# tum-vision/mem

Hardware: AMD Instinct MI355X
Metric: pretrain samples/sec (ViT-B, 224^2 event voxels) (higher is better)
Workload: dtype bf16; 1 GPU; MEM pretrain ViT-Base/16, 224^2 2-bin event voxels, bf16, batch 256 per GPU (BASELINE configs[1]); step = rasterize 256x30k events + event_norm + masks + ViT fwd/CE/bwd + clip + AdamW; global_batch=256, parallelism=dp1, stochastic_depth=work skipping, optimizer=AdamW as one launch in front of the next forward, last_block_mlp_rows=rows that reach the head

## Files before the change

include/memhip.h:

```cpp
#ifndef MEMHIP_H
#define MEMHIP_H

#include <stddef.h>
#include <stdint.h>

#ifdef __cplusplus
extern "C" {
#endif

#define MEMHIP_ABI_VERSION 10

#define MEMHIP_OK 0
#define MEMHIP_EINVAL (-1)
#define MEMHIP_EWORKSPACE (-2)
#define MEMHIP_ELAUNCH (-3)
#define MEMHIP_EUNSUPPORTED (-4)

typedef void* memhip_stream_t;

int memhip_abi_version(void);
const char* memhip_last_error(void);
const char* memhip_arch(void);
const char* memhip_build_flags(void);
int memhip_set_option(const char* name, int value);
int memhip_get_option(const char* name, int* value);
int memhip_stream_reserve_cus(memhip_stream_t stream, int cus);


typedef struct memhip_event_aug {
  double scale_x, scale_y;
  int32_t time_flip;
  int32_t flip_x;
  int64_t flip_w;
  int32_t shift_x, shift_y;
  int32_t do_filter;
  int32_t filt_w, filt_h;
  int32_t infer;
} memhip_event_aug_t;
#define MEMHIP_AUG_INFER_FLIP_W 1
#define MEMHIP_AUG_INFER_FILT_W 2
#define MEMHIP_AUG_INFER_FILT_H 4

enum { MEMHIP_RASTER_AUTO = 0, MEMHIP_RASTER_SINGLE = 1, MEMHIP_RASTER_BINNED = 2,
       MEMHIP_RASTER_LDS = 3, MEMHIP_RASTER_GLOBAL = 4, MEMHIP_RASTER_GLOBAL_VAR = 5 };
typedef struct memhip_raster_args {
  const double* ev;
  const int64_t* offsets;
  const memhip_event_aug_t* aug;
  const int32_t* dims;
  int32_t B, H, W, time_surface;
  int32_t form;
  int32_t reserved0;
  int64_t n_events;
  uint8_t* out;
  int32_t* status;
  void* workspace;
  size_t workspace_bytes;
} memhip_raster_args_t;
int memhip_rasterize(const memhip_raster_args_t* args, memhip_stream_t stream);

enum { MEMHIP_RASTER_K_COUNT,
       MEMHIP_RASTER_K_FINALIZE,
       MEMHIP_RASTER_K_LDS,
       MEMHIP_RASTER_K_BIN_KEYS,
       MEMHIP_RASTER_K_BIN_ACCUM };
typedef struct memhip_raster_launch {
  int32_t kernel;
  int32_t grid_x, grid_y;
  int32_t block;
  int32_t lds;
} memhip_raster_launch_t;
typedef struct memhip_raster_plan {
  int32_t family;
  int32_t rows_per_band, bands;
  int32_t band_px, nb;
  int32_t bx;
  uint64_t ws_bytes;
  uint64_t off_bins, off_tstat;
  uint64_t off_keys, off_hdr, off_bad_slots;
  uint64_t clear_ws_bytes, clear_status_bytes, clear_out_bytes;
  int32_t count;
  memhip_raster_launch_t l[2];
} memhip_raster_plan_t;
int memhip_rasterize_plan(const memhip_raster_args_t* args, int device_cus, memhip_raster_plan_t* out);

int memhip_aug_resolve(const double* extent, memhip_event_aug_t* aug, int B, int stage, int fixed_h, int fixed_w,
                       int hmax, int wmax, int32_t* dims, int32_t* status, memhip_stream_t stream);

int memhip_events_extent(const double* ev, const int64_t* offsets, const memhip_event_aug_t* aug,
                         int B, double* extent, memhip_stream_t stream);

#define MEMHIP_DT_U8 0
#define MEMHIP_DT_I8 1
#define MEMHIP_DT_U16 2
#define MEMHIP_DT_I16 3
#define MEMHIP_DT_U32 4
#define MEMHIP_DT_I32 5
#define MEMHIP_DT_U64 6
#define MEMHIP_DT_I64 7
#define MEMHIP_DT_F32 8
#define MEMHIP_DT_F64 9
#define MEMHIP_DT_BOOL 10
int memhip_decode_ncaltech101(const uint8_t* raw, int64_t n_bytes, double* ev, memhip_stream_t stream);
int memhip_events_from_columns(const void* x, int x_dtype, const void* y, int y_dtype, const void* t, int t_dtype,
                               const void* p, int p_dtype, int64_t n, double* ev, memhip_stream_t stream);
size_t memhip_events_dsec_workspace(int64_t n);
int memhip_events_dsec(const void* in, int dtype, int64_t n, double y_limit, double* out, int64_t* n_out,
                       void* workspace, size_t workspace_bytes, memhip_stream_t stream);

int memhip_resample_to_f32(const uint8_t* in, const int32_t* dims, int64_t slot_bytes, int fixed_h, int fixed_w, int mode,
                           const int32_t* offs, int B, int OH, int OW, float* out, memhip_stream_t stream);
int memhip_to_uint8(const float* x, int64_t n, uint8_t* y, memhip_stream_t stream);
int memhip_rand_augment_u8(const uint8_t* in, uint8_t* out, const void* ops, int B, int H, int W, memhip_stream_t stream);
int memhip_color_jitter(const void* in, int in_is_u8, int B, int H, int W, const void* params, float* out, int out_chans,
                        memhip_stream_t stream);

#define MEMHIP_EV_RM_TS 1
#define MEMHIP_EV_HOTPIX 2
#define MEMHIP_EV_LOG 4
#define MEMHIP_EV_GAMMA 8
#define MEMHIP_EV_NORMALIZE 16
int memhip_event_norm(const void* in, int in_is_u8, int B, int H, int W, int flags,
                      float num_stds, float gamma, float* out, int out_chans,
                      memhip_stream_t stream);
int memhip_event_norm_topk(const void* in, int in_is_u8, int B, int H, int W, int flags,
                           int num_hot_pixels, float gamma, float* out, int out_chans,
                           uint64_t* hot_keys, memhip_stream_t stream);

int memhip_mt_seed(uint32_t* mt_state, const uint32_t* key, int key_len);
double memhip_mt_random(uint32_t* mt_state);
int memhip_mask_blockwise(uint32_t* mt_state, int H, int W, int num_masking_patches,
                          int min_num_patches, int max_num_patches, double log_aspect_lo,
                          double log_aspect_hi, int n_masks, uint8_t* out);
int memhip_mask_random_location(uint32_t* mt_state, int H, int W, int num_masking_patches,
                                int n_masks, uint8_t* out);

#define MEMHIP_EPI_BIAS_BF16 0
#define MEMHIP_EPI_BIAS_GELU 1
#define MEMHIP_EPI_RESIDUAL 2
#define MEMHIP_EPI_DGELU 3
#define MEMHIP_EPI_F32 4
#define MEMHIP_EPI_PATCH_EMBED 5
#define MEMHIP_EPI_BIAS_GELU_DG 6
#define MEMHIP_EPI_MUL_AUX 7
#define MEMHIP_EPI_RESIDUAL_DROP 8

typedef struct memhip_dropout {
  uint32_t key0, key1;
  uint32_t site;
  uint32_t thr;
  float scale;
  int32_t row0;
} memhip_dropout_t;
int memhip_dropout_mask(const memhip_dropout_t* d, int row0, int rows, int cols, uint8_t* out, memhip_stream_t stream);
int memhip_dropout_rows_f32(const memhip_dropout_t* d, float* x, int64_t ldx, int rows, int D, memhip_stream_t stream);

typedef struct memhip_gemm_args {
  const void* A; const void* B;
  int64_t lda, ldb;
  int32_t M, N, K, epilogue;
  void* out0; int64_t ldo0;
  void* out1; int64_t ldo1;
  const float* bias;
  const float* vec1;
  float* resid; int64_t ldr;
  const void* aux; int64_t ldaux;
  const float* rowmask;
  float keep_prob;
  float colscale; int32_t colscale_n;
  int32_t rows_per_sample;
  int32_t accumulate;
  float* colsum;
  const int32_t* sample_map;
  int32_t colsum_copies;
  int32_t reserved0;
  const memhip_dropout_t* dropout;
} memhip_gemm_args_t;
int memhip_gemm_bf16_nt(const memhip_gemm_args_t* args, memhip_stream_t stream);

#define MEMHIP_NT_128 0
#define MEMHIP_NT_G256 1
#define MEMHIP_NT_P8_256 2
#define MEMHIP_NT_P8_128 3
#define MEMHIP_NT_P8_PAIR 4
typedef struct memhip_nt_launch {
  int32_t kind;
  int32_t row0, rows;
  int32_t tail_rows;
  int32_t guard;
  int32_t copy;
  int32_t grid, tail_grid;
} memhip_nt_launch_t;
typedef struct memhip_nt_plan { int32_t count; memhip_nt_launch_t l[2]; } memhip_nt_plan_t;
int memhip_gemm_bf16_nt_plan(const memhip_gemm_args_t* args, int stream_cus, int device_cus, memhip_nt_plan_t* out);

size_t memhip_gemm_bf16_tn_workspace(int R, int N, int K);
int memhip_gemm_bf16_tn(const void* A, int64_t lda, const void* B, int64_t ldb, int R, int N, int K,
                        float* out, int64_t ldo, int accumulate, void* workspace, size_t workspace_bytes,
                        memhip_stream_t stream);
typedef struct memhip_tn_problem {
  const void* A; int64_t lda;
  const void* B; int64_t ldb;
  float* out; int64_t ldo;
  int32_t R, N, K;
  int32_t reserved0;
} memhip_tn_problem_t;
size_t memhip_gemm_bf16_tn_group_workspace(const memhip_tn_problem_t* problems, int count);
int memhip_gemm_bf16_tn_group(const memhip_tn_problem_t* problems, int count, int accumulate, void* workspace,
                              size_t workspace_bytes, memhip_stream_t stream);

#define MEMHIP_TN_128 0
#define MEMHIP_TN_P8_ATOMIC 1
#define MEMHIP_TN_P8_WS 2
#define MEMHIP_TN_P8_GROUP 3
typedef struct memhip_tn_part {
  int32_t problem;
  int32_t tiles, splits, rows_per_split;
  int32_t wg_begin, quad_begin;
  int64_t ws_offset;
} memhip_tn_part_t;
typedef struct memhip_tn_launch {
  int32_t kind;
  int32_t count;
  int32_t grid, reduce_grid;
  int32_t memset_first;
  int32_t use_atomics;
  int64_t ws_bytes;
  memhip_tn_part_t p[4];
} memhip_tn_launch_t;
typedef struct memhip_tn_plan { int32_t count; int32_t reserved0; memhip_tn_launch_t l[4]; } memhip_tn_plan_t;
int memhip_gemm_bf16_tn_plan(const memhip_tn_problem_t* problems, int count, int accumulate, const void* workspace,
                             size_t workspace_bytes, int stream_cus, memhip_tn_plan_t* out_plan);
size_t memhip_gemm_bf16_tn_plan_workspace(const memhip_tn_problem_t* problems, int count, int device_cus);
int memhip_colsum_bf16(const void* in, int64_t ld, int R, int C, float* out, memhip_stream_t stream);
int memhip_colsum_fold(float* ws, int copies, int N, float* out, memhip_stream_t stream);

int memhip_residual_rows(const float* x, int64_t ldx, const int32_t* rows, const void* y, int64_t ldy, const float* gamma,
                         const float* rowkeep, float keep_prob, int R, int D, float* out, int64_t ldo,
                         memhip_stream_t stream);
int memhip_scatter_rows_f32(const float* src, int64_t lds, const int32_t* rows, int R, int D, float* dst, int64_t ldd,
                            memhip_stream_t stream);

int memhip_layernorm_fwd(const float* x, int64_t ldx, const int32_t* row_idx, int R, int D,
                         const float* gamma, const float* beta, float eps, void* y_bf16, int64_t ldy,
                         float* mean, float* rstd, memhip_stream_t stream);
int memhip_layernorm_bwd(const void* dy_bf16, int64_t lddy, const float* x, int64_t ldx,
                         const int32_t* row_idx, int R, int D, const float* gamma, const float* mean,
                         const float* rstd, float* dres, int64_t lddres, int accumulate, float* dgamma,
                         float* dbeta, memhip_stream_t stream);

int memhip_layerscale_grad(const void* W_bf16, int64_t ldw, const float* dW, int64_t lddw, const float* bias,
                           const float* dbias, const float* gamma, int N, int K, float* dgamma,
                           memhip_stream_t stream);

typedef struct memhip_branch {
  const void* y; int64_t ldy;
  const float* gamma;
  const float* rowmask;
  float keep_prob;
  int32_t rows_per_sample;
  void* dy; int64_t lddy;
  float* dgamma; float* dbias;
  const int32_t* out_map;
  const memhip_dropout_t* dropout;
} memhip_branch_t;
typedef struct memhip_branch_bwd_args {
  const float* dx; int64_t lddx;
  int32_t M, D;
  memhip_branch_t branch;
} memhip_branch_bwd_args_t;
int memhip_branch_bwd(const memhip_branch_bwd_args_t* args, memhip_stream_t stream);
typedef struct memhip_ln_bwd_branch_args {
  const void* dy; int64_t lddy;
  const float* x; int64_t ldx;
  int32_t R, D;
  const float* gamma; const float* mean; const float* rstd;
  float* dres; int64_t lddres;
  float* dgamma; float* dbeta;
  const int32_t* in_map;
  memhip_branch_t branch;
} memhip_ln_bwd_branch_args_t;
int memhip_layernorm_bwd_branch(const memhip_ln_bwd_branch_args_t* args, memhip_stream_t stream);

int memhip_embed_bwd(const float* dx, int64_t lddx, const uint8_t* mask, int B, int L, int D,
                     void* dy_bf16, int64_t lddy, float* dcls, float* dmask_token, memhip_stream_t stream);

int memhip_cross_entropy(void* logits_bf16, int64_t ld, const int64_t* labels, int M, int V,
                         float grad_scale, float* row_loss, int32_t* row_correct, int write_grad,
                         float* out2, memhip_stream_t stream);

int memhip_attn_tokens_padded(int T);
int memhip_relpos_gather(const float* table, const int32_t* index , int T, int TP, int heads,
                         float* bias_pad, float* biasT_pad ,
                         memhip_stream_t stream);
int memhip_attn_fwd(const void* qkv, int64_t ldqkv, int B, int T, int D, int heads, const float* table,
                    int window_h, int window_w, void* out, int64_t ldo, float* lse, memhip_stream_t stream);
int memhip_attn_delta(const void* dout, const void* out, int64_t ldo, int64_t rows, int heads, float* delta,
                      memhip_stream_t stream);
typedef struct memhip_attn_bwd_args {
  const void* qkv; int64_t ldqkv;
  const void* dout; int64_t ldo;
  const void* out; int64_t ldout;
  const float* lse;
  float* delta;
  const float* table;
  int32_t window_h, window_w, B, T, D, heads;
  float scale;
  int32_t reserved0;
  void* dqkv; int64_t lddqkv;
  float* dtable; float* dq_bias; float* dv_bias;
  void* ws; int64_t ws_bytes;
} memhip_attn_bwd_args_t;
int memhip_attn_bwd(const memhip_attn_bwd_args_t* args, memhip_stream_t stream);
int64_t memhip_attn_bwd_workspace(int B, int T, int heads, int window_h, int window_w);

#define MEMHIP_ATTN_16 1
#define MEMHIP_ATTN_SMALL 2
#define MEMHIP_ATTN_WIN 3
#define MEMHIP_ATTN_WIN_DS 4
#define MEMHIP_ATTN_STREAM 5
enum { MEMHIP_ATTN_K_STATS_ZERO, MEMHIP_ATTN_K_DELTA, MEMHIP_ATTN_K_FWD, MEMHIP_ATTN_K_BWD_KV, MEMHIP_ATTN_K_BWD_Q,
       MEMHIP_ATTN_K_FWD16, MEMHIP_ATTN_K_BWD16,
       MEMHIP_ATTN_K_WIN_STATS, MEMHIP_ATTN_K_FWD_WIN, MEMHIP_ATTN_K_BWD_KV_WIN, MEMHIP_ATTN_K_BWD_Q_WIN,
       MEMHIP_ATTN_K_BWD_KVS_WIN, MEMHIP_ATTN_K_BWD_QS_WIN,
       MEMHIP_ATTN_K_FWD_STREAM, MEMHIP_ATTN_K_BWD_KV_STREAM, MEMHIP_ATTN_K_BWD_Q_STREAM };
typedef struct memhip_attn_launch {
  int32_t kernel;
  int32_t grid_x, grid_y, grid_z;
  int32_t block;
  int32_t lds;
} memhip_attn_launch_t;
typedef struct memhip_attn_plan {
  int32_t family;
  int32_t n;
  int32_t ww;
  int32_t vb, dt, fd;
  int32_t spb;
  int32_t nwg;
  int32_t groups;
  int32_t nbz, nbq, nbs;
  int32_t qgroups, qs;
  int32_t stream_spb;
  int32_t lds_over;
  int32_t count;
  memhip_attn_launch_t l[5];
} memhip_attn_plan_t;
int memhip_attn_plan_fwd(int B, int T, int D, int heads, int window_h, int window_w, int stream_cus, memhip_attn_plan_t* out);
int memhip_attn_plan_bwd(int B, int T, int D, int heads, int window_h, int window_w, int has_dtable, int has_dv_bias,
                         int has_out, const void* ws, int64_t ws_bytes, int stream_cus, memhip_attn_plan_t* out);

int memhip_f32_gemm_nt(const memhip_gemm_args_t* args, memhip_stream_t stream);
int memhip_f32_transpose(const float* in, int64_t ldin, int R, int C, float* out, int64_t ldout, memhip_stream_t stream);
int memhip_f32_layernorm_fwd(const float* x, int64_t ldx, const int32_t* row_idx, int R, int D, const float* gamma,
                             const float* beta, float eps, float* y, int64_t ldy, float* mean, float* rstd,
                             memhip_stream_t stream);
int memhip_f32_layernorm_bwd(const float* dy, int64_t lddy, const float* x, int64_t ldx, const int32_t* row_idx, int R, int D,
                             const float* gamma, const float* mean, const float* rstd, float* dres, int64_t lddres,
                             int accumulate, float* dgamma, float* dbeta, memhip_stream_t stream);
int memhip_f32_branch_bwd(const float* dx, int64_t lddx, const float* y, int64_t ldy, const float* gamma, const float* rowmask,
                          float keep_prob, int rows_per_sample, int M, int D, float* dy, int64_t lddy, float* dgamma,
                          float* dbias, memhip_stream_t stream);
int memhip_f32_embed_bwd(const float* dx, int64_t lddx, const uint8_t* mask, int B, int L, int D, float* dy, int64_t lddy,
                         float* dcls, float* dmask_token, memhip_stream_t stream);
int memhip_f32_cross_entropy(float* logits, int64_t ld, const int64_t* labels, int M, int V, float grad_scale,
                             float* row_loss, int32_t* row_correct, int write_grad, float* out2, memhip_stream_t stream);
int memhip_f32_colsum(const float* in, int64_t ld, int R, int C, float* out, memhip_stream_t stream);
int memhip_f32_im2col(const float* x, int B, int C, int H, int W, int ph, int pw, float* out, memhip_stream_t stream);
int memhip_f32_attn_fwd(const float* qkv, int64_t ldqkv, int B, int T, int D, int heads, const float* table,
                        const int32_t* index, float* out, int64_t ldo, float* lse, memhip_stream_t stream);
int memhip_f32_attn_bwd(const float* qkv, int64_t ldqkv, const float* dout, int64_t ldo, int B, int T, int D, int heads,
                        float scale, const float* table, const int32_t* index, float* dqkv, int64_t lddqkv, float* dtable,
                        memhip_stream_t stream);

int memhip_mae_enc_assemble(const float* xe, const float* pos, const float* cls, const int64_t* ids_keep, int B, int L, int K,
                            int D, float* out, memhip_stream_t stream);
int memhip_mae_enc_assemble_bwd(const float* dx, const int64_t* ids_keep, int B, int L, int K, int D, float* dxe, float* dcls,
                                memhip_stream_t stream);
int memhip_mae_dec_assemble(const float* y, const float* mask_token, const float* dpos, const int64_t* ids_restore, int B, int L,
                            int K, int D, float* out, memhip_stream_t stream);
int memhip_mae_dec_assemble_bwd(const float* dxd, const int64_t* ids_restore, int B, int L, int K, int D, float* dy,
                                float* dmask_token, memhip_stream_t stream);
int memhip_mae_loss(const float* pred, const float* img, const float* mask, int B, int C, int H, int W, int patch,
                    int only_masked, float* row_loss, float* dpred, float* scratch2, memhip_stream_t stream);

enum { MEMHIP_CONV_BF16, MEMHIP_CONV_F32, MEMHIP_CONV_F16X2 };
typedef struct memhip_conv_args {
  int32_t mode;
  int32_t reserved0;
  const void* in;
  int64_t in_plane;
  const void* weight;
  int64_t w_plane;
  const float* bias;
  const void* add;
  int64_t add_plane;
  void* out;
  int64_t out_plane;
  int32_t B, H, W, Cin, Cout, ksize, stride, pad;
  int32_t relu;
  int32_t out_padded;
  int32_t out_f32;
  int32_t reserved1;
  const int32_t* n_active;
} memhip_conv_args_t;
int memhip_conv2d_nhwc(const memhip_conv_args_t* args, memhip_stream_t stream);
int memhip_nchw_to_padded_nhwc4(const float* x, int B, int C, int H, int W, const float* mean, const float* stdv, void* out,
// ... 281 lines not shown
```

mem_amd/csrc/fp32_path.hip:

```cpp
#include "common.h"
#include "gemm_epilogue.hpp"

namespace {

using namespace memhip;

typedef __attribute__((ext_vector_type(4))) float f32x4;

__device__ __forceinline__ float wsumf(float v) {
  for (int o = 32; o > 0; o >>= 1) v += __shfl_xor(v, o);
  return v;
}
__device__ __forceinline__ float wmaxf(float v) {
  for (int o = 32; o > 0; o >>= 1) v = fmaxf(v, __shfl_xor(v, o));
  return v;
}
__device__ __forceinline__ float gelu_exact(float x) { return 0.5f * x * (1.0f + erff(x * 0.70710678118654752440f)); }
__device__ __forceinline__ float gelu_grad_exact(float x) {
  const float cdf = 0.5f * (1.0f + erff(x * 0.70710678118654752440f));
  return cdf + x * expf(-0.5f * x * x) * 0.39894228040143267794f;
}

constexpr int BM = 128, BN = 128, BK = 32, kThreads = 256, PITCH = BK + 2;
constexpr int kTileFloats = BM * PITCH, kStageFloats = 2 * kTileFloats;
// ... 247 lines not shown
  s = wsumf(s);
  const int lab = (int)labels[r];
  const float lse = logf(s) + mx;
  if (lane == 0) { row_loss[r] = lse - l[lab]; row_ok[r] = am == lab; }
  if (write_grad)
    for (int c = lane; c < V; c += 64) l[c] = (expf(l[c] - lse) - (c == lab ? 1.0f : 0.0f)) * grad_scale;
}
__global__ __launch_bounds__(256) void ce_reduce_f32_kernel(const float* __restrict__ row_loss, const int* __restrict__ row_ok, int M,
                                                            float* __restrict__ out2) {
  __shared__ double sl[256]; __shared__ int so[256];
  double s = 0.0; int k = 0;
  for (int i = threadIdx.x; i < M; i += 256) { s += row_loss[i]; k += row_ok[i]; }
  sl[threadIdx.x] = s; so[threadIdx.x] = k;
  __syncthreads();
  if (threadIdx.x == 0) {
    double t = 0; int q = 0;
    for (int i = 0; i < 256; ++i) { t += sl[i]; q += so[i]; }
    out2[0] = (float)(t / M); out2[1] = (float)q / (float)M;
  }
}

__global__ __launch_bounds__(256) void colsum_f32_kernel(const float* __restrict__ in, long long ld, int R, int Cc, float* __restrict__ out) {
  const int c = blockIdx.x * 256 + threadIdx.x;
  if (c >= Cc) return;
  float s = 0.f;
  for (int r = blockIdx.y; r < R; r += gridDim.y) s += in[(long long)r * ld + c];
  atomicAdd(out + c, s);
}

__global__ __launch_bounds__(256) void im2col_f32_kernel(const float* __restrict__ x, int B, int C, int H, int W, int ph, int pw,
                                                         float* __restrict__ out) {
  const int gh = H / ph, gw = W / pw, K = C * ph * pw;
  const long long total = (long long)B * gh * gw * K;
  for (long long i = (long long)blockIdx.x * 256 + threadIdx.x; i < total; i += (long long)gridDim.x * 256) {
    const int k = (int)(i % K);
    const long long row = i / K;
    const int px = k % pw, py = (k / pw) % ph, c = k / (pw * ph);
    const int gx = (int)(row % gw), gy = (int)((row / gw) % gh), b = (int)(row / ((long long)gw * gh));
    out[i] = x[(((long long)b * C + c) * H + gy * ph + py) * W + gx * pw + px];
  }
}

constexpr int kMaxKeys = 4;

template <int HD>
__global__ __launch_bounds__(256) void attn_fwd_f32_kernel(const float* __restrict__ qkv, long long ld, int B, int T, int D, int heads,
                                                           const float* __restrict__ table, const int* __restrict__ index,
                                                           float* __restrict__ out, long long ldo, float* __restrict__ lse) {
  const int bh = blockIdx.x, b = bh / heads, h = bh - b * heads;
  const int i = blockIdx.y * 4 + (threadIdx.x >> 6), lane = threadIdx.x & 63;
  if (i >= T) return;
  const float* q = qkv + ((long long)b * T + i) * ld + h * HD;
  float s[kMaxKeys];
  float mx = -INFINITY;
#pragma unroll
  for (int u = 0; u < kMaxKeys; ++u) {
    const int j = lane + u * 64;
    s[u] = -INFINITY;
    if (j < T) {
      const float* k = qkv + ((long long)b * T + j) * ld + D + h * HD;
      float a = 0.f;
      for (int d = 0; d < HD; ++d) a += q[d] * k[d];
      if (index) a += table[(long long)index[i * T + j] * heads + h];
      s[u] = a;
      mx = fmaxf(mx, a);
    }
  }
  mx = wmaxf(mx);
  float sum = 0.f;
#pragma unroll
  for (int u = 0; u < kMaxKeys; ++u) { s[u] = (lane + u * 64 < T) ? expf(s[u] - mx) : 0.f; sum += s[u]; }
  sum = wsumf(sum);
  const float inv = 1.0f / sum;
  for (int d = 0; d < HD; ++d) {
    float a = 0.f;
#pragma unroll
    for (int u = 0; u < kMaxKeys; ++u) {
      const int j = lane + u * 64;
      if (j < T) a += s[u] * inv * qkv[((long long)b * T + j) * ld + 2 * D + h * HD + d];
    }
    a = wsumf(a);
    if (lane == 0) out[((long long)b * T + i) * ldo + h * HD + d] = a;
  }
  if (lane == 0 && lse) lse[((long long)b * heads + h) * T + i] = logf(sum) + mx;
}

template <int HD>
__global__ __launch_bounds__(256) void attn_bwd_f32_kernel(const float* __restrict__ qkv, long long ld, const float* __restrict__ dout,
                                                           long long ldo, int B, int T, int D, int heads, float scale,
                                                           const float* __restrict__ table, const int* __restrict__ index,
                                                           float* __restrict__ dqkv, long long ldd, float* __restrict__ dtable) {
  const int bh = blockIdx.x, b = bh / heads, h = bh - b * heads;
  const int i = blockIdx.y * 4 + (threadIdx.x >> 6), lane = threadIdx.x & 63;
  if (i >= T) return;
  const float* q = qkv + ((long long)b * T + i) * ld + h * HD;
  const float* dO = dout + ((long long)b * T + i) * ldo + h * HD;
  float p[kMaxKeys], dp[kMaxKeys];
  float mx = -INFINITY;
#pragma unroll
  for (int u = 0; u < kMaxKeys; ++u) {
    const int j = lane + u * 64;
    p[u] = -INFINITY; dp[u] = 0.f;
    if (j < T) {
      const float* k = qkv + ((long long)b * T + j) * ld + D + h * HD;
      const float* v = qkv + ((long long)b * T + j) * ld + 2 * D + h * HD;
      float a = 0.f, g = 0.f;
      for (int d = 0; d < HD; ++d) { a += q[d] * k[d]; g += dO[d] * v[d]; }
      if (index) a += table[(long long)index[i * T + j] * heads + h];
      p[u] = a; dp[u] = g;
      mx = fmaxf(mx, a);
    }
  }
  mx = wmaxf(mx);
  float sum = 0.f;
#pragma unroll
  for (int u = 0; u < kMaxKeys; ++u) { p[u] = (lane + u * 64 < T) ? expf(p[u] - mx) : 0.f; sum += p[u]; }
  sum = wsumf(sum);
  float delta = 0.f;
#pragma unroll
  for (int u = 0; u < kMaxKeys; ++u) { p[u] /= sum; delta += p[u] * dp[u]; }
  delta = wsumf(delta);
  float ds[kMaxKeys];
#pragma unroll
  for (int u = 0; u < kMaxKeys; ++u) {
    const int j = lane + u * 64;
    ds[u] = p[u] * (dp[u] - delta);
    if (j < T) {
      if (dtable && index) atomicAdd(dtable + (long long)index[i * T + j] * heads + h, ds[u]);
      float* dk = dqkv + ((long long)b * T + j) * ldd + D + h * HD;
      float* dv = dqkv + ((long long)b * T + j) * ldd + 2 * D + h * HD;
      for (int d = 0; d < HD; ++d) { atomicAdd(dk + d, ds[u] * q[d]); atomicAdd(dv + d, p[u] * dO[d]); }
    }
  }
  for (int d = 0; d < HD; ++d) {
    float a = 0.f;
#pragma unroll
    for (int u = 0; u < kMaxKeys; ++u) {
      const int j = lane + u * 64;
      if (j < T) a += ds[u] * qkv[((long long)b * T + j) * ld + D + h * HD + d];
    }
    a = wsumf(a);
    if (lane == 0) dqkv[((long long)b * T + i) * ldd + h * HD + d] = a * scale;
  }
}

}

extern "C" int memhip_f32_gemm_nt(const memhip_gemm_args_t* a, memhip_stream_t stream) {
  MEMHIP_REQUIRE(a, "gemm_f32: null args");
  GemmArgs p;
  __builtin_memset(&p, 0, sizeof(p));
  __builtin_memcpy(&p, a, offsetof(memhip_gemm_args_t, dropout));
  if (a->dropout) return fail(MEMHIP_EUNSUPPORTED, "gemm_f32: dropout is not part of the fp32 parity path");
  MEMHIP_REQUIRE(p.M >= 0 && p.N > 0 && p.K > 0, "gemm_f32: bad shape M=%d N=%d K=%d", p.M, p.N, p.K);
  if (p.M == 0) return MEMHIP_OK;
  MEMHIP_REQUIRE(p.A && p.B && p.K % 4 == 0 && p.lda % 4 == 0 && p.ldb % 4 == 0 && ((uintptr_t)p.A & 15) == 0 &&
                     ((uintptr_t)p.B & 15) == 0,
                 "gemm_f32: operands must be 16-byte aligned with K and ld multiples of 4");
  hipStream_t s = as_stream(stream);
  switch (p.epilogue) {
    case MEMHIP_EPI_BIAS_BF16: MEMHIP_REQUIRE(p.out0, "gemm_f32: out0"); return launch_f32<MEMHIP_EPI_BIAS_BF16>(p, s);
    case MEMHIP_EPI_BIAS_GELU: MEMHIP_REQUIRE(p.out0 && p.out1, "gemm_f32: out0/out1"); return launch_f32<MEMHIP_EPI_BIAS_GELU>(p, s);
    case MEMHIP_EPI_RESIDUAL: MEMHIP_REQUIRE(p.resid, "gemm_f32: residual args"); return launch_f32<MEMHIP_EPI_RESIDUAL>(p, s);
    case MEMHIP_EPI_DGELU: MEMHIP_REQUIRE(p.out0 && p.aux, "gemm_f32: dgelu args"); return launch_f32<MEMHIP_EPI_DGELU>(p, s);
    case MEMHIP_EPI_F32: MEMHIP_REQUIRE(p.out0, "gemm_f32: out0"); return launch_f32<MEMHIP_EPI_F32>(p, s);
    case MEMHIP_EPI_PATCH_EMBED: MEMHIP_REQUIRE(p.resid && p.vec1 && p.aux, "gemm_f32: patch args"); return launch_f32<MEMHIP_EPI_PATCH_EMBED>(p, s);
    default: return fail(MEMHIP_EUNSUPPORTED, "gemm_f32: epilogue %d is not part of the fp32 path", p.epilogue);
  }
}

extern "C" int memhip_f32_transpose(const float* in, int64_t ldin, int R, int Cc, float* out, int64_t ldout, memhip_stream_t stream) {
  MEMHIP_REQUIRE(R >= 0 && Cc > 0 && ldout >= R, "transpose_f32: bad shape");
  if (R == 0) return MEMHIP_OK;
  MEMHIP_REQUIRE(in && out, "transpose_f32: null pointer");
  hipLaunchKernelGGL(transpose_f32_kernel, dim3(cdiv(Cc, 32), cdiv(ldout, 32)), dim3(256), 0, as_stream(stream), in, (long long)ldin,
                     R, Cc, out, (long long)ldout);
  return check_launch("transpose_f32");
}

extern "C" int memhip_f32_layernorm_fwd(const float* x, int64_t ldx, const int32_t* row_idx, int R, int D, const float* gamma,
                                        const float* beta, float eps, float* y, int64_t ldy, float* mean, float* rstd,
                                        memhip_stream_t stream) {
  MEMHIP_REQUIRE(R >= 0 && D > 0, "ln_fwd_f32: bad shape");
  if (R == 0) return MEMHIP_OK;
  MEMHIP_REQUIRE(x && gamma && beta && y && mean && rstd, "ln_fwd_f32: null pointer");
  hipLaunchKernelGGL(ln_fwd_f32_kernel, dim3(cdiv(R, 4)), dim3(256), 0, as_stream(stream), x, (long long)ldx, row_idx, R, D, gamma,
                     beta, eps, y, (long long)ldy, mean, rstd);
  return check_launch("ln_fwd_f32");
}

extern "C" int memhip_f32_layernorm_bwd(const float* dy, int64_t lddy, const float* x, int64_t ldx, const int32_t* row_idx, int R,
                                        int D, const float* gamma, const float* mean, const float* rstd, float* dres,
                                        int64_t lddres, int accumulate, float* dgamma, float* dbeta, memhip_stream_t stream) {
  MEMHIP_REQUIRE(R >= 0 && D > 0, "ln_bwd_f32: bad shape");
  if (R == 0) return MEMHIP_OK;
  MEMHIP_REQUIRE(dy && x && gamma && mean && rstd && dres && dgamma && dbeta, "ln_bwd_f32: null pointer");
  hipLaunchKernelGGL(ln_bwd_f32_kernel, dim3(cdiv(R, 4)), dim3(256), 0, as_stream(stream), dy, (long long)lddy, x, (long long)ldx,
                     row_idx, R, D, gamma, mean, rstd, dres, (long long)lddres, accumulate, dgamma, dbeta);
  return check_launch("ln_bwd_f32");
}

extern "C" int memhip_f32_branch_bwd(const float* dx, int64_t lddx, const float* y, int64_t ldy, const float* gamma,
                                     const float* rowmask, float keep_prob, int rows_per_sample, int M, int D, float* dy,
                                     int64_t lddy, float* dgamma, float* dbias, memhip_stream_t stream) {
  MEMHIP_REQUIRE(M >= 0 && D > 0 && rows_per_sample > 0, "branch_bwd_f32: bad shape");
  if (M == 0) return MEMHIP_OK;
  MEMHIP_REQUIRE(dx && dy, "branch_bwd_f32: null pointer");
  hipLaunchKernelGGL(branch_bwd_f32_kernel, dim3(cdiv(M, 4)), dim3(256), 0, as_stream(stream), dx, (long long)lddx, y, (long long)ldy,
                     gamma, rowmask, keep_prob, rows_per_sample, M, D, dy, (long long)lddy, dgamma, dbias);
  return check_launch("branch_bwd_f32");
}

extern "C" int memhip_f32_embed_bwd(const float* dx, int64_t lddx, const uint8_t* mask, int B, int L, int D, float* dy,
                                    int64_t lddy, float* dcls, float* dmask_token, memhip_stream_t stream) {
  MEMHIP_REQUIRE(B >= 0 && L > 0 && D > 0, "embed_bwd_f32: bad shape");
  if (B == 0) return MEMHIP_OK;
  MEMHIP_REQUIRE(dx && mask && dy && dcls && dmask_token, "embed_bwd_f32: null pointer");
  hipLaunchKernelGGL(embed_bwd_f32_kernel, dim3(B), dim3(256), 0, as_stream(stream), dx, (long long)lddx, mask, B, L, D, dy,
                     (long long)lddy, dcls, dmask_token);
  return check_launch("embed_bwd_f32");
}

extern "C" int memhip_f32_cross_entropy(float* logits, int64_t ld, const int64_t* labels, int M, int V, float grad_scale,
                                        float* row_loss, int32_t* row_correct, int write_grad, float* out2,
                                        memhip_stream_t stream) {
  MEMHIP_REQUIRE(M > 0 && V > 0, "ce_f32: bad shape");
  MEMHIP_REQUIRE(logits && labels && row_loss && row_correct && out2, "ce_f32: null pointer");
  hipStream_t s = as_stream(stream);
  hipLaunchKernelGGL(ce_f32_kernel, dim3(cdiv(M, 4)), dim3(256), 0, s, logits, (long long)ld, (const long long*)labels, M, V,
                     grad_scale, row_loss, row_correct, write_grad);
  hipLaunchKernelGGL(ce_reduce_f32_kernel, dim3(1), dim3(256), 0, s, row_loss, row_correct, M, out2);
  return check_launch("ce_f32");
}

extern "C" int memhip_f32_colsum(const float* in, int64_t ld, int R, int C, float* out, memhip_stream_t stream) {
  MEMHIP_REQUIRE(R >= 0 && C > 0, "colsum_f32: bad shape");
  if (R == 0) return MEMHIP_OK;
  MEMHIP_REQUIRE(in && out, "colsum_f32: null pointer");
  const int gy = R < 64 ? 1 : 64;
  hipLaunchKernelGGL(colsum_f32_kernel, dim3(cdiv(C, 256), gy), dim3(256), 0, as_stream(stream), in, (long long)ld, R, C, out);
  return check_launch("colsum_f32");
}

extern "C" int memhip_f32_im2col(const float* x, int B, int C, int H, int W, int ph, int pw, float* out, memhip_stream_t stream) {
  MEMHIP_REQUIRE(B >= 0 && C > 0 && H % ph == 0 && W % pw == 0, "im2col_f32: bad shape");
  if (B == 0) return MEMHIP_OK;
  MEMHIP_REQUIRE(x && out, "im2col_f32: null pointer");
  hipLaunchKernelGGL(im2col_f32_kernel, dim3(2048), dim3(256), 0, as_stream(stream), x, B, C, H, W, ph, pw, out);
  return check_launch("im2col_f32");
}

extern "C" int memhip_f32_attn_fwd(const float* qkv, int64_t ldqkv, int B, int T, int D, int heads, const float* table,
                                   const int32_t* index, float* out, int64_t ldo, float* lse, memhip_stream_t stream) {
  MEMHIP_REQUIRE(B >= 0 && T > 0 && T <= 64 * kMaxKeys && heads > 0 && D % heads == 0, "attn_f32: bad shape (T <= 256)");
  if (B == 0) return MEMHIP_OK;
  MEMHIP_REQUIRE(qkv && out && (!index || table), "attn_f32: null pointer");
  const int hd = D / heads;
  dim3 grid(B * heads, cdiv(T, 4));
  hipStream_t s = as_stream(stream);
  if (hd == 64) hipLaunchKernelGGL(attn_fwd_f32_kernel<64>, grid, dim3(256), 0, s, qkv, (long long)ldqkv, B, T, D, heads, table, index, out, (long long)ldo, lse);
  else if (hd == 32) hipLaunchKernelGGL(attn_fwd_f32_kernel<32>, grid, dim3(256), 0, s, qkv, (long long)ldqkv, B, T, D, heads, table, index, out, (long long)ldo, lse);
  else return fail(MEMHIP_EUNSUPPORTED, "attn_f32: head_dim %d (32 or 64)", hd);
  return check_launch("attn_fwd_f32");
}

extern "C" int memhip_f32_attn_bwd(const float* qkv, int64_t ldqkv, const float* dout, int64_t ldo, int B, int T, int D, int heads,
                                   float scale, const float* table, const int32_t* index, float* dqkv, int64_t lddqkv,
                                   float* dtable, memhip_stream_t stream) {
  MEMHIP_REQUIRE(B >= 0 && T > 0 && T <= 64 * kMaxKeys && heads > 0 && D % heads == 0, "attn_bwd_f32: bad shape (T <= 256)");
  if (B == 0) return MEMHIP_OK;
  MEMHIP_REQUIRE(qkv && dout && dqkv && (!index || table), "attn_bwd_f32: null pointer");
  const int hd = D / heads;
  dim3 grid(B * heads, cdiv(T, 4));
  hipStream_t s = as_stream(stream);
  MEMHIP_HIP(hipMemset2DAsync(dqkv, (size_t)lddqkv * 4, 0, (size_t)3 * D * 4, (size_t)B * T, s));
  if (hd == 64) hipLaunchKernelGGL(attn_bwd_f32_kernel<64>, grid, dim3(256), 0, s, qkv, (long long)ldqkv, dout, (long long)ldo, B, T, D, heads, scale, table, index, dqkv, (long long)lddqkv, dtable);
  else if (hd == 32) hipLaunchKernelGGL(attn_bwd_f32_kernel<32>, grid, dim3(256), 0, s, qkv, (long long)ldqkv, dout, (long long)ldo, B, T, D, heads, scale, table, index, dqkv, (long long)lddqkv, dtable);
  else return fail(MEMHIP_EUNSUPPORTED, "attn_bwd_f32: head_dim %d (32 or 64)", hd);
  return check_launch("attn_bwd_f32");
}

namespace {

__global__ __launch_bounds__(256) void mae_enc_assemble_kernel(const float* __restrict__ xe, const float* __restrict__ pos,
                                                               const float* __restrict__ cls, const long long* __restrict__ ids_keep,
                                                               int B, int L, int K, int D, float* __restrict__ out) {
  const int row = blockIdx.x;
  const int b = row / (K + 1), t = row - b * (K + 1);
  float* o = out + (long long)row * D;
  if (t == 0) {
    for (int c = threadIdx.x; c < D; c += 256) o[c] = cls[c] + pos[c];
  } else {
    const long long l = ids_keep[(long long)b * K + t - 1];
    const float* s = xe + ((long long)b * L + l) * D;
    const float* p = pos + (1 + l) * D;
    for (int c = threadIdx.x; c < D; c += 256) o[c] = s[c] + p[c];
  }
}
__global__ __launch_bounds__(256) void mae_enc_assemble_bwd_kernel(const float* __restrict__ dx, const long long* __restrict__ ids_keep,
                                                                   int B, int L, int K, int D, float* __restrict__ dxe,
                                                                   float* __restrict__ dcls) {
  const int row = blockIdx.x;
  const int b = row / (K + 1), t = row - b * (K + 1);
  const float* g = dx + (long long)row * D;
  if (t == 0) {
    for (int c = threadIdx.x; c < D; c += 256) atomicAdd(dcls + c, g[c]);
// ... 126 lines not shown
```

mem_amd/csrc/gemm.hip:

```cpp
#include <cstddef>
#include "common.h"
#include "gemm_epilogue.hpp"

namespace {

using namespace memhip;

constexpr int BM = 128, BN = 128, BK = 64;
constexpr int kThreads = 256;
constexpr int kTileBytes = BM * BK * 2;
constexpr int kStageBytes = 2 * kTileBytes;

typedef __attribute__((ext_vector_type(8))) __bf16 bf16x8;
typedef __attribute__((ext_vector_type(4))) float f32x4;

__device__ __forceinline__ int swz_slot(int row, int chunk) { return row * 8 + (chunk ^ ((row >> 1) & 7)); }

__device__ __forceinline__ void glds16(const void* gsrc, void* lds_dst) {
  __builtin_amdgcn_global_load_lds((const __attribute__((address_space(1))) void*)gsrc,
                                   (__attribute__((address_space(3))) void*)lds_dst, 16, 0, 0);
}

__device__ __forceinline__ void stage_tile(const __bf16* __restrict__ src, long long ld, int row0,
                                           int rows_valid, int k0, char* lds_tile, int wave, int lane) {
#pragma unroll
  for (int j = 0; j < 4; ++j) {
    const int inst = wave * 4 + j;
    const int row = inst * 8 + (lane >> 3);
    const int cpos = lane & 7;
    const int chunk = cpos ^ ((row >> 1) & 7);
    int grow = row0 + row;
    grow = grow < rows_valid ? grow : rows_valid - 1;
    const __bf16* g = src + (long long)grow * ld + k0 + chunk * 8;
    glds16(g, lds_tile + inst * 1024);
  }
}

template <int EPI>
__global__ __launch_bounds__(kThreads, 2) void gemm_nt_kernel(typename EpiArgs<EPI>::type p) {
  extern __shared__ __attribute__((aligned(16))) char smem[];
  const int lane = threadIdx.x & 63;
  const int wave = __builtin_amdgcn_readfirstlane(threadIdx.x >> 6);
  const int wr = wave >> 1, wc = wave & 1;

  const int nwg = gridDim.x;
  int pid = blockIdx.x;
  {
    const int q = nwg >> 3, r = nwg & 7, xcd = pid & 7, idx = pid >> 3;
    pid = (xcd < r ? xcd * (q + 1) : r * (q + 1) + (xcd - r) * q) + idx;
  }
  const int ntn = (p.N + BN - 1) / BN;
  const int tile_m = pid / ntn, tile_n = pid % ntn;
  const int m0 = tile_m * BM, n0 = tile_n * BN;

  f32x4 acc[4][4];
#pragma unroll
  for (int i = 0; i < 4; ++i)
#pragma unroll
    for (int j = 0; j < 4; ++j) acc[i][j] = f32x4{0.f, 0.f, 0.f, 0.f};

  const int nk = p.K / BK;
  stage_tile(p.A, p.lda, m0, p.M, 0, smem, wave, lane);
  stage_tile(p.B, p.ldb, n0, p.N, 0, smem + kTileBytes, wave, lane);
  __syncthreads();

  int cur = 0;
  for (int t = 0; t < nk; ++t) {
    if (t + 1 < nk) {
      char* nxt = smem + (cur ^ 1) * kStageBytes;
      stage_tile(p.A, p.lda, m0, p.M, (t + 1) * BK, nxt, wave, lane);
      stage_tile(p.B, p.ldb, n0, p.N, (t + 1) * BK, nxt + kTileBytes, wave, lane);
    }
    const char* At = smem + cur * kStageBytes;
    const char* Bt = At + kTileBytes;
#pragma unroll
    for (int kk = 0; kk < 2; ++kk) {
      bf16x8 af[4], bfr[4];
      const int chunk = kk * 4 + (lane >> 4);
#pragma unroll
      for (int i = 0; i < 4; ++i) {
        const int row = wr * 64 + i * 16 + (lane & 15);
        af[i] = *reinterpret_cast<const bf16x8*>(At + swz_slot(row, chunk) * 16);
      }
#pragma unroll
      for (int j = 0; j < 4; ++j) {
        const int row = wc * 64 + j * 16 + (lane & 15);
        bfr[j] = *reinterpret_cast<const bf16x8*>(Bt + swz_slot(row, chunk) * 16);
      }
#pragma unroll
      for (int i = 0; i < 4; ++i)
#pragma unroll
        for (int j = 0; j < 4; ++j)
          acc[i][j] = __builtin_amdgcn_mfma_f32_16x16x32_bf16(af[i], bfr[j], acc[i][j], 0, 0, 0);
    }
    __syncthreads();
    cur ^= 1;
  }

  const int mw = m0 + wr * 64, nw = n0 + wc * 64;
  if (vec_ok(p) && nw + 64 <= p.N) {
    constexpr int LS = 72;
    float* wreg = reinterpret_cast<float*>(smem + wave * 16384);
    float cs[8] = {0.f, 0.f, 0.f, 0.f, 0.f, 0.f, 0.f, 0.f};
    EpiCols cols;
    epi_cols_load<EPI>(p, nw + (lane & 7) * 8, cols);
#pragma unroll
    for (int half = 0; half < 2; ++half) {
#pragma unroll
      for (int ii = 0; ii < 2; ++ii)
#pragma unroll
        for (int j = 0; j < 4; ++j)
#pragma unroll
          for (int r = 0; r < 4; ++r)
            wreg[(ii * 16 + (lane >> 4) * 4 + r) * LS + j * 16 + (lane & 15)] = acc[half * 2 + ii][j][r];
#pragma unroll
      for (int it = 0; it < 4; ++it) {
        const int row = it * 8 + (lane >> 3), c8 = (lane & 7) * 8;
        const int m = mw + half * 32 + row;
        float v[8];
        ld8(wreg + row * LS + c8, v);
        if (m < p.M) epilogue8<EPI>(p, m, nw + c8, v, cs, cols);
      }
    }
    colsum_flush(p, nw + (lane & 7) * 8, cs, lane);
    return;
  }
  float bias_n[4], vec_n[4];
#pragma unroll
  for (int j = 0; j < 4; ++j) {
    const int n = n0 + wc * 64 + j * 16 + (lane & 15);
    const int nc = n < p.N ? n : p.N - 1;
    bias_n[j] = p.bias ? p.bias[nc] : 0.f;
    vec_n[j] = p.vec1 ? p.vec1[nc] : 0.f;
  }
#pragma unroll
  for (int i = 0; i < 4; ++i) {
#pragma unroll
    for (int r = 0; r < 4; ++r) {
      const int m = m0 + wr * 64 + i * 16 + (lane >> 4) * 4 + r;
      if (m >= p.M) continue;
#pragma unroll
      for (int j = 0; j < 4; ++j) {
        const int n = n0 + wc * 64 + j * 16 + (lane & 15);
        if (n < p.N) epilogue<EPI>(p, m, n, acc[i][j][r], bias_n[j], vec_n[j]);
      }
    }
  }
}

template <int EPI>
int launch(const GemmArgs& p, hipStream_t s, int grid) {
  static bool attr_done = false;
  if (!attr_done) {
    hipError_t e = hipFuncSetAttribute(reinterpret_cast<const void*>(gemm_nt_kernel<EPI>),
                                       hipFuncAttributeMaxDynamicSharedMemorySize, 2 * kStageBytes);
    if (e != hipSuccess) return fail(MEMHIP_ELAUNCH, "gemm: set smem attr: %s", hipGetErrorString(e));
    attr_done = true;
  }
  hipLaunchKernelGGL(gemm_nt_kernel<EPI>, dim3(grid), dim3(kThreads), 2 * kStageBytes, s,
                     static_cast<const typename EpiArgs<EPI>::type&>(p));
  return check_launch("gemm_bf16_nt");
}

int validate(const memhip_gemm_args_t* a, GemmArgsD& p) {
  MEMHIP_REQUIRE(a, "gemm: null args");
  static_assert(offsetof(GemmArgs, m_base) == offsetof(memhip_gemm_args_t, dropout),
                "GemmArgs = the ABI struct up to `dropout` + internal tail");
  __builtin_memset(&p, 0, sizeof(p));
  __builtin_memcpy(&p, a, offsetof(memhip_gemm_args_t, dropout));
  MEMHIP_REQUIRE(p.M >= 0 && p.N > 0 && p.K > 0, "gemm: bad shape M=%d N=%d K=%d", p.M, p.N, p.K);
  if (p.M == 0) return MEMHIP_OK;
  MEMHIP_REQUIRE(p.K % BK == 0, "gemm: K=%d must be a multiple of %d", p.K, BK);
  MEMHIP_REQUIRE(p.A && p.B, "gemm: null operand");
  MEMHIP_REQUIRE(p.lda % 8 == 0 && p.ldb % 8 == 0 && ((uintptr_t)p.A & 15) == 0 && ((uintptr_t)p.B & 15) == 0,
                 "gemm: operands must be 16-byte aligned with ld %% 8 == 0");
  switch (p.epilogue) {
    case MEMHIP_EPI_BIAS_BF16: MEMHIP_REQUIRE(p.out0, "gemm: out0"); break;
    case MEMHIP_EPI_BIAS_GELU: MEMHIP_REQUIRE(p.out0 && p.out1, "gemm: out0/out1"); break;
    case MEMHIP_EPI_RESIDUAL:
      MEMHIP_REQUIRE(p.resid, "gemm: residual args");
      MEMHIP_REQUIRE(!p.sample_map || (!p.rowmask && p.rows_per_sample > 0), "gemm: sample_map excludes rowmask");
      break;
    case MEMHIP_EPI_DGELU: MEMHIP_REQUIRE(p.out0 && p.aux, "gemm: dgelu args"); break;
    case MEMHIP_EPI_BIAS_GELU_DG: MEMHIP_REQUIRE(p.out0 && p.out1, "gemm: out0/out1"); break;
    case MEMHIP_EPI_MUL_AUX: MEMHIP_REQUIRE(p.out0 && p.aux, "gemm: mul_aux args"); break;
    case MEMHIP_EPI_F32: MEMHIP_REQUIRE(p.out0, "gemm: out0"); break;
    case MEMHIP_EPI_PATCH_EMBED: MEMHIP_REQUIRE(p.resid && p.vec1 && p.aux, "gemm: patch args"); break;
    case MEMHIP_EPI_RESIDUAL_DROP:
      MEMHIP_REQUIRE(p.resid && a->dropout, "gemm: residual-dropout args (resid, dropout)");
      MEMHIP_REQUIRE(!p.out0, "gemm: the residual-dropout epilogue writes no bf16 branch copy (out0 must be NULL)");
      MEMHIP_REQUIRE(p.N % 8 == 0, "gemm: residual-dropout epilogue needs N %% 8 == 0 (N=%d)", p.N);
      MEMHIP_REQUIRE(!p.sample_map || (!p.rowmask && p.rows_per_sample > 0), "gemm: sample_map excludes rowmask");
      p.drop = drop_params(*a->dropout);
      break;
    default: return fail(MEMHIP_EINVAL, "gemm: unknown epilogue %d", p.epilogue);
  }
  MEMHIP_REQUIRE(!a->dropout || p.epilogue == MEMHIP_EPI_RESIDUAL_DROP, "gemm: dropout is taken by epilogue %d only",
                 MEMHIP_EPI_RESIDUAL_DROP);
  return MEMHIP_OK;
}

NtPlan plan_now(const GemmArgs& p, int stream_cus, int device_cus) {
  if (p.M == 0) return NtPlan{};
  const NtOptions o = {opt(OPT_GEMM_P8), opt(OPT_GEMM256), opt(OPT_GEMM_SPLIT), opt(OPT_GEMM_P8_HALF), opt(OPT_GEMM_P8_PAIR),
                       opt(OPT_GEMM_P8_MIN_N), opt(OPT_GEMM256_MIN_N)};
  return gemm_nt_plan(p, stream_cus, device_cus, o);
}

GemmArgsD slice_rows(GemmArgsD p, int row0, int rows) {
  const long long r = row0;
  p.A += r * p.lda;
  if (p.out0) p.out0 = (char*)p.out0 + r * p.ldo0 * (p.epilogue == MEMHIP_EPI_F32 ? 4 : 2);
  if (p.out1) p.out1 = (char*)p.out1 + r * p.ldo1 * 2;
  if (p.resid && !p.sample_map) p.resid += r * p.ldr;
  if (p.aux && !(p.sample_map && epi_resid(p.epilogue)))
    p.aux = (const char*)p.aux + r * p.ldaux * (epi_resid(p.epilogue) ? 4 : 2);
  p.M = rows;
  p.m_base = row0;
  return p;
}

}

namespace memhip {
int gemm256_launch(const GemmArgs& p, const NtLaunch& l, hipStream_t s);
int gemm_p8_launch(const GemmArgs& p, const NtLaunch& l, hipStream_t s);
int gemm_p8_pair_launch(const GemmArgs& head, const GemmArgs& tail, const NtLaunch& l, hipStream_t s);
}

extern "C" int memhip_gemm_bf16_nt(const memhip_gemm_args_t* a, memhip_stream_t stream) {
  GemmArgsD p;
  if (const int rc = validate(a, p)) return rc;
  hipStream_t s = as_stream(stream);
  const NtPlan plan = plan_now(p, usable_cus(s), max_cus());
  for (int i = 0; i < plan.count; ++i) {
    const NtLaunch& l = plan.l[i];
    const GemmArgsD part = slice_rows(p, l.row0, l.rows);
    int rc;
    switch (l.kind) {
      case MEMHIP_NT_P8_PAIR: rc = gemm_p8_pair_launch(part, slice_rows(p, l.row0 + l.rows, l.tail_rows), l, s); break;
      case MEMHIP_NT_P8_256:
      case MEMHIP_NT_P8_128: rc = gemm_p8_launch(part, l, s); break;
      case MEMHIP_NT_G256: rc = gemm256_launch(part, l, s); break;
      default:
        rc = dispatch_epilogue(part.epilogue, [&](auto E) { return launch<decltype(E)::value>(part, s, l.grid); });
    }
    if (rc != MEMHIP_OK) return rc;
  }
  return MEMHIP_OK;
}

extern "C" int memhip_gemm_bf16_nt_plan(const memhip_gemm_args_t* a, int stream_cus, int device_cus, memhip_nt_plan_t* out) {
  MEMHIP_REQUIRE(out && stream_cus >= 0 && device_cus >= 0, "gemm plan: bad arguments");
  GemmArgsD p;
  if (const int rc = validate(a, p)) return rc;
  *out = plan_now(p, stream_cus, device_cus);
  return MEMHIP_OK;
}
```

mem_amd/csrc/gemm_epilogue.hpp:

```cpp
#pragma once
#include <type_traits>
#include "common.h"
#include "dropout.hpp"
#include "gemm_nt_plan.hpp"

namespace memhip {

struct GemmArgsD : GemmArgs {
  DropParams drop;
};
__host__ __device__ __forceinline__ const DropParams& drop_of(const GemmArgs& p) { return static_cast<const GemmArgsD&>(p).drop; }

constexpr bool epi_resid(int e) { return e == MEMHIP_EPI_RESIDUAL || e == MEMHIP_EPI_RESIDUAL_DROP; }
template <int EPI> struct EpiArgs { typedef GemmArgs type; };
template <> struct EpiArgs<MEMHIP_EPI_RESIDUAL_DROP> { typedef GemmArgsD type; };

template <class F>
int dispatch_epilogue(int epi, F&& f) {
  switch (epi) {
#define MEMHIP_EPI_CASE(E) case E: return f(std::integral_constant<int, E>{})
    MEMHIP_EPI_CASE(MEMHIP_EPI_BIAS_BF16);
    MEMHIP_EPI_CASE(MEMHIP_EPI_BIAS_GELU);
    MEMHIP_EPI_CASE(MEMHIP_EPI_RESIDUAL);
    MEMHIP_EPI_CASE(MEMHIP_EPI_DGELU);
    MEMHIP_EPI_CASE(MEMHIP_EPI_F32);
    MEMHIP_EPI_CASE(MEMHIP_EPI_PATCH_EMBED);
    MEMHIP_EPI_CASE(MEMHIP_EPI_BIAS_GELU_DG);
    MEMHIP_EPI_CASE(MEMHIP_EPI_MUL_AUX);
    MEMHIP_EPI_CASE(MEMHIP_EPI_RESIDUAL_DROP);
#undef MEMHIP_EPI_CASE
    default: return fail(MEMHIP_EINVAL, "gemm: unknown epilogue %d", epi);
  }
}

__device__ __forceinline__ unsigned drop_row(const GemmArgs& p, long long rr) {
  return (unsigned)(drop_of(p).row0 + rr + (p.sample_map ? 0 : p.m_base));
}

__device__ __forceinline__ float bf16_round(float v) { return (float)(__bf16)v; }

__device__ __forceinline__ float* colsum_base(const GemmArgs& p) {
  return p.colsum_copies > 1 ? p.colsum + (long long)((int)blockIdx.x % p.colsum_copies) * p.N : p.colsum;
}

__device__ __forceinline__ float erf_fast(float x) {
  const float ax = fabsf(x);
  const float t = __frcp_rn(fmaf(0.3275911f, ax, 1.0f));
  float poly = fmaf(1.061405429f, t, -1.453152027f);
  poly = fmaf(poly, t, 1.421413741f);
  poly = fmaf(poly, t, -0.284496736f);
  poly = fmaf(poly, t, 0.254829592f);
  const float y = 1.0f - poly * t * __expf(-ax * ax);
  return copysignf(y, x);
}

__device__ __forceinline__ float gelu_f(float x) {
  return x * 0.5f * (1.0f + erf_fast(x * 0.70710678118654752440f));
}
__device__ __forceinline__ float gelu_grad_f(float x) {
  const float cdf = 0.5f * (1.0f + erf_fast(x * 0.70710678118654752440f));
  const float pdf = __expf(-0.5f * x * x) * 0.39894228040143267794f;
  return cdf + x * pdf;
}

template <int EPI>
__device__ __forceinline__ void epilogue(const GemmArgs& p, int m, int n, float acc, float bias_n,
                                         float vec_n) {
  if constexpr (EPI == MEMHIP_EPI_BIAS_BF16) {
    float v = acc + bias_n;
    __bf16 y = (__bf16)v;
    if (n < p.colscale_n) y = (__bf16)((float)y * p.colscale);
    reinterpret_cast<__bf16*>(p.out0)[(long long)m * p.ldo0 + n] = y;
    if (p.colsum) atomicAdd(colsum_base(p) + n, (float)y);
  } else if constexpr (EPI == MEMHIP_EPI_BIAS_GELU) {
    const __bf16 h = (__bf16)(acc + bias_n);
    reinterpret_cast<__bf16*>(p.out0)[(long long)m * p.ldo0 + n] = h;
    reinterpret_cast<__bf16*>(p.out1)[(long long)m * p.ldo1 + n] = (__bf16)gelu_f((float)h);
  } else if constexpr (EPI == MEMHIP_EPI_BIAS_GELU_DG) {
    const __bf16 h = (__bf16)(acc + bias_n);
    reinterpret_cast<_Float16*>(p.out0)[(long long)m * p.ldo0 + n] = (_Float16)gelu_grad_f((float)h);
    reinterpret_cast<__bf16*>(p.out1)[(long long)m * p.ldo1 + n] = (__bf16)gelu_f((float)h);
  } else if constexpr (EPI == MEMHIP_EPI_MUL_AUX) {
    const float da = bf16_round(acc);
    const float g = (float)reinterpret_cast<const _Float16*>(p.aux)[(long long)m * p.ldaux + n];
    const __bf16 o = (__bf16)(da * g);
    reinterpret_cast<__bf16*>(p.out0)[(long long)m * p.ldo0 + n] = o;
    if (p.colsum) atomicAdd(colsum_base(p) + n, (float)o);
  } else if constexpr (EPI == MEMHIP_EPI_RESIDUAL) {
    const __bf16 y = (__bf16)(acc + bias_n);
    if (p.out0) reinterpret_cast<__bf16*>(p.out0)[(long long)m * p.ldo0 + n] = y;
    float t = p.vec1 ? __fmul_rn(vec_n, (float)y) : (float)y;
    if (p.rowmask) t = __fmul_rn(__fdiv_rn(t, p.keep_prob), p.rowmask[(m + p.m_base) / p.rows_per_sample]);
    long long rr = m;
    if (p.sample_map) {
      const int mm = m + p.m_base, c = mm / p.rows_per_sample;
      rr = (long long)p.sample_map[c] * p.rows_per_sample + (mm - c * p.rows_per_sample);
      t = __fdiv_rn(t, p.keep_prob);
    }
    const float xin = p.aux ? reinterpret_cast<const float*>(p.aux)[rr * p.ldaux + n] : p.resid[rr * p.ldr + n];
    p.resid[rr * p.ldr + n] = __fadd_rn(xin, t);
  } else if constexpr (EPI == MEMHIP_EPI_RESIDUAL_DROP) {
    const __bf16 y = (__bf16)(acc + bias_n);
    long long rr = m;
    if (p.sample_map) {
      const int mm = m + p.m_base, c = mm / p.rows_per_sample;
      rr = (long long)p.sample_map[c] * p.rows_per_sample + (mm - c * p.rows_per_sample);
    }
    const DropParams& d = drop_of(p);
    const float z = __fmul_rn((float)y, dropout_mul(d, dropout_keep8(d, drop_row(p, rr), (unsigned)(n >> 3)), n & 7));
    float t = p.vec1 ? __fmul_rn(vec_n, z) : z;
    if (p.rowmask) t = __fmul_rn(__fdiv_rn(t, p.keep_prob), p.rowmask[(m + p.m_base) / p.rows_per_sample]);
    if (p.sample_map) t = __fdiv_rn(t, p.keep_prob);
    const float xin = p.aux ? reinterpret_cast<const float*>(p.aux)[rr * p.ldaux + n] : p.resid[rr * p.ldr + n];
    p.resid[rr * p.ldr + n] = __fadd_rn(xin, t);
  } else if constexpr (EPI == MEMHIP_EPI_DGELU) {
    const float da = bf16_round(acc);
    const float h = (float)reinterpret_cast<const __bf16*>(p.aux)[(long long)m * p.ldaux + n];
    const __bf16 o = (__bf16)(da * gelu_grad_f(h));
    reinterpret_cast<__bf16*>(p.out0)[(long long)m * p.ldo0 + n] = o;
    if (p.colsum) atomicAdd(colsum_base(p) + n, (float)o);
  } else if constexpr (EPI == MEMHIP_EPI_F32) {
    float* o = reinterpret_cast<float*>(p.out0) + (long long)m * p.ldo0 + n;
    *o = p.accumulate ? (*o + acc) : acc;
  } else if constexpr (EPI == MEMHIP_EPI_PATCH_EMBED) {
    const float y = bf16_round(acc + bias_n);
    const int L = p.rows_per_sample;
    const int b = m / L, pi = m - b * L;
    const float w = (float)reinterpret_cast<const unsigned char*>(p.aux)[m];
    const float v = __fadd_rn(__fmul_rn(y, 1.0f - w), __fmul_rn(vec_n, w));
    p.resid[((long long)b * (L + 1) + 1 + pi) * p.ldr + n] = v;
  }
}


typedef __attribute__((ext_vector_type(8))) __bf16 ebf16x8;
typedef __attribute__((ext_vector_type(2))) __bf16 ebf16x2;
typedef __attribute__((ext_vector_type(2))) float ef32x2;

__device__ __forceinline__ void ld8(const float* p, float* o) {
  const float4 a = reinterpret_cast<const float4*>(p)[0], b = reinterpret_cast<const float4*>(p)[1];
  o[0] = a.x; o[1] = a.y; o[2] = a.z; o[3] = a.w; o[4] = b.x; o[5] = b.y; o[6] = b.z; o[7] = b.w;
}
__device__ __forceinline__ void st8(float* p, const float* o) {
  reinterpret_cast<float4*>(p)[0] = float4{o[0], o[1], o[2], o[3]};
  reinterpret_cast<float4*>(p)[1] = float4{o[4], o[5], o[6], o[7]};
}

__device__ __forceinline__ unsigned pack_bf16x2(ef32x2 v) {
  return __builtin_bit_cast(unsigned, __builtin_convertvector(v, ebf16x2));
}
__device__ __forceinline__ ef32x2 unpack_bf16x2(unsigned u) {
  return ef32x2{__uint_as_float(u << 16), __uint_as_float(u & 0xffff0000u)};
}
typedef __attribute__((ext_vector_type(2))) _Float16 ef16x2;
__device__ __forceinline__ unsigned pack_f16x2(ef32x2 v) {
  return __builtin_bit_cast(unsigned, __builtin_convertvector(v, ef16x2));
}
__device__ __forceinline__ ef32x2 unpack_f16x2(unsigned u) {
  return __builtin_convertvector(__builtin_bit_cast(ef16x2, u), ef32x2);
}
__device__ __forceinline__ ef32x2 fma2(ef32x2 a, ef32x2 b, ef32x2 c) { return __builtin_elementwise_fma(a, b, c); }
__device__ __forceinline__ ef32x2 splat2(float v) { return ef32x2{v, v}; }

typedef __attribute__((ext_vector_type(4))) unsigned eu32x4;
__device__ __forceinline__ void st_stream16(void* base, long long elem_off, unsigned a, unsigned b, unsigned c, unsigned d) {
  __builtin_nontemporal_store(eu32x4{a, b, c, d}, reinterpret_cast<eu32x4*>(reinterpret_cast<__bf16*>(base) + elem_off));
}

__device__ __forceinline__ void erf_exp2(ef32x2 x, ef32x2& erf, ef32x2& e) {
  const ef32x2 z = x * splat2(0.70710678118654752440f);
  const ef32x2 az = __builtin_elementwise_abs(z);
  const ef32x2 d = fma2(splat2(0.3275911f), az, splat2(1.0f));
  const ef32x2 t = ef32x2{__builtin_amdgcn_rcpf(d.x), __builtin_amdgcn_rcpf(d.y)};
  ef32x2 poly = fma2(splat2(1.061405429f), t, splat2(-1.453152027f));
  poly = fma2(poly, t, splat2(1.421413741f));
  poly = fma2(poly, t, splat2(-0.284496736f));
  poly = fma2(poly, t, splat2(0.254829592f));
  const ef32x2 w = az * az * splat2(-1.4426950408889634f);
  e = ef32x2{__builtin_amdgcn_exp2f(w.x), __builtin_amdgcn_exp2f(w.y)};
  const ef32x2 y = fma2(-(poly * t), e, splat2(1.0f));
  erf = ef32x2{copysignf(y.x, z.x), copysignf(y.y, z.y)};
}
__device__ __forceinline__ ef32x2 gelu2(ef32x2 x) {
  ef32x2 erf, e;
  erf_exp2(x, erf, e);
  const ef32x2 hx = x * splat2(0.5f);
  return fma2(hx, erf, hx);
}
__device__ __forceinline__ void gelu_and_grad2(ef32x2 x, ef32x2& g, ef32x2& dg) {
  ef32x2 erf, e;
  erf_exp2(x, erf, e);
  const ef32x2 hx = x * splat2(0.5f);
  g = fma2(hx, erf, hx);
  const ef32x2 cdf = fma2(splat2(0.5f), erf, splat2(0.5f));
  dg = fma2(x * splat2(0.39894228040143267794f), e, cdf);
}
__device__ __forceinline__ ef32x2 gelu_grad2(ef32x2 x) {
  ef32x2 erf, e;
  erf_exp2(x, erf, e);
  const ef32x2 cdf = fma2(splat2(0.5f), erf, splat2(0.5f));
  return fma2(x * splat2(0.39894228040143267794f), e, cdf);
}

struct EpiCols {
  ef32x2 bias[4];
  float g[8];
};
static __device__ __attribute__((aligned(32))) const float g_epi_zero8[8] = {0.f, 0.f, 0.f, 0.f, 0.f, 0.f, 0.f, 0.f};
static __device__ __attribute__((aligned(32))) const float g_epi_one8[8] = {1.f, 1.f, 1.f, 1.f, 1.f, 1.f, 1.f, 1.f};
static __device__ __attribute__((aligned(128))) const float g_epi_zero256[256] = {};
struct EpiOnes256 { float v[256]; constexpr EpiOnes256() : v() { for (int i = 0; i < 256; ++i) v[i] = 1.0f; } };
static __device__ __attribute__((aligned(128))) const EpiOnes256 g_epi_one256_s{};
#define g_epi_one256 (g_epi_one256_s.v)
typedef const float __attribute__((address_space(1)))* gcf32_ptr;
typedef float __attribute__((ext_vector_type(4))) ef32x4;
typedef const ef32x4 __attribute__((address_space(1)))* gcf32x4_ptr;
__device__ __forceinline__ gcf32_ptr as_global(const float* q) { return (gcf32_ptr)q; }
__device__ __forceinline__ void ld8g(gcf32_ptr q, float* o) {
  const ef32x4 a = reinterpret_cast<gcf32x4_ptr>(q)[0], b = reinterpret_cast<gcf32x4_ptr>(q)[1];
  o[0] = a[0]; o[1] = a[1]; o[2] = a[2]; o[3] = a[3]; o[4] = b[0]; o[5] = b[1]; o[6] = b[2]; o[7] = b[3];
}
template <int EPI>
__device__ __forceinline__ void epi_cols_load(const GemmArgs& p, int n, EpiCols& c) {
  if constexpr (EPI != MEMHIP_EPI_DGELU && EPI != MEMHIP_EPI_F32 && EPI != MEMHIP_EPI_MUL_AUX) {
    float b[8];
    ld8g(p.bias ? as_global(p.bias + n) : as_global(g_epi_zero8), b);
#pragma unroll
    for (int k = 0; k < 4; ++k) c.bias[k] = ef32x2{b[2 * k], b[2 * k + 1]};
  }
  if constexpr (epi_resid(EPI)) {
    ld8g(p.vec1 ? as_global(p.vec1 + n) : as_global(g_epi_one8), c.g);
  }
}

template <int EPI>
struct EpiRow {};
template <>
struct EpiRow<MEMHIP_EPI_DGELU> { uint4 h; };
template <>
struct EpiRow<MEMHIP_EPI_MUL_AUX> { uint4 h; };
template <>
struct EpiRow<MEMHIP_EPI_RESIDUAL> { float x[8]; float rm; long long row; };
template <>
struct EpiRow<MEMHIP_EPI_RESIDUAL_DROP> : EpiRow<MEMHIP_EPI_RESIDUAL> {};
__device__ const float g_epi_one = 1.0f;
__device__ const int g_epi_izero = 0;
typedef const int __attribute__((address_space(1)))* gci32_ptr;
__device__ __attribute__((aligned(256))) unsigned char g_epi_trash[1024];
template <int EPI, bool BIGROWS = true>
__device__ __forceinline__ void epi_row_load(const GemmArgs& p, int m, int n, EpiRow<EPI>& r) {
  if constexpr (EPI == MEMHIP_EPI_DGELU || EPI == MEMHIP_EPI_MUL_AUX) {
    r.h = *reinterpret_cast<const uint4*>(reinterpret_cast<const __bf16*>(p.aux) + (long long)m * p.ldaux + n);
  } else if constexpr (epi_resid(EPI)) {
    const float* base = p.aux ? reinterpret_cast<const float*>(p.aux) : p.resid;
    const long long ld = p.aux ? p.ldaux : p.ldr;
    const int mm = m + p.m_base;
    const bool per_sample = p.rowmask || p.sample_map;
    const float inv = per_sample ? __frcp_rn((float)p.rows_per_sample) : 0.f;
    int smp = (int)(((float)mm + 0.5f) * inv);
    if constexpr (BIGROWS) {
      if (per_sample && mm >= (1 << 21)) smp = mm / p.rows_per_sample;
    }
    const gcf32_ptr rmb = p.rowmask ? as_global(p.rowmask) : as_global(&g_epi_one);
    r.rm = rmb[p.rowmask ? smp : 0];
    const gci32_ptr smb = p.sample_map ? (gci32_ptr)p.sample_map : (gci32_ptr)&g_epi_izero;
    const int kid = smb[p.sample_map ? smp : 0];
    r.row = p.sample_map ? (long long)kid * p.rows_per_sample + (mm - smp * p.rows_per_sample) : (long long)m;
    ld8(base + r.row * ld + n, r.x);
  }
}

typedef eu32x4 __attribute__((address_space(1)))* gu32x4_ptr;
__device__ __forceinline__ void st_branch_copy(const GemmArgs& p, int m, int n, const unsigned* y) {
  const gu32x4_ptr dst = p.out0 ? (gu32x4_ptr)(reinterpret_cast<__bf16*>(p.out0) + (long long)m * p.ldo0 + n)
                                : (gu32x4_ptr)(g_epi_trash + 2 * (n & 255));
  *dst = eu32x4{y[0], y[1], y[2], y[3]};
}

template <int EPI> struct EpiPk { static constexpr int W = 4; };
template <> struct EpiPk<MEMHIP_EPI_BIAS_GELU> { static constexpr int W = 8; };
template <> struct EpiPk<MEMHIP_EPI_BIAS_GELU_DG> { static constexpr int W = 8; };
template <> struct EpiPk<MEMHIP_EPI_RESIDUAL> { static constexpr int W = 8; };
template <> struct EpiPk<MEMHIP_EPI_RESIDUAL_DROP> { static constexpr int W = 8; };
template <> struct EpiPk<MEMHIP_EPI_F32> { static constexpr int W = 8; };
template <> struct EpiPk<MEMHIP_EPI_PATCH_EMBED> { static constexpr int W = 8; };

template <int EPI, int COPY = 1>
__device__ __forceinline__ void epi8_math(const GemmArgs& p, int m, int n, const float* acc, float* cs, const EpiCols& c,
                                          const EpiRow<EPI>& row, unsigned* out) {
  ef32x2 t[4];
#pragma unroll
  for (int k = 0; k < 4; ++k) t[k] = ef32x2{acc[2 * k], acc[2 * k + 1]};
  if constexpr (EPI != MEMHIP_EPI_DGELU && EPI != MEMHIP_EPI_F32 && EPI != MEMHIP_EPI_MUL_AUX) {
#pragma unroll
    for (int k = 0; k < 4; ++k) t[k] += c.bias[k];
  }
  if constexpr (EPI == MEMHIP_EPI_BIAS_BF16) {
    unsigned y[4];
#pragma unroll
    for (int k = 0; k < 4; ++k) y[k] = pack_bf16x2(t[k]);
    if (p.colscale_n > 0 && n < p.colscale_n) {
#pragma unroll
      for (int k = 0; k < 4; ++k) y[k] = pack_bf16x2(unpack_bf16x2(y[k]) * splat2(p.colscale));
    }
    if (p.colsum) {
#pragma unroll
      for (int k = 0; k < 4; ++k) {
        const ef32x2 f = unpack_bf16x2(y[k]);
        cs[2 * k] += f.x;
        cs[2 * k + 1] += f.y;
      }
    }
#pragma unroll
    for (int k = 0; k < 4; ++k) out[k] = y[k];
  } else if constexpr (EPI == MEMHIP_EPI_BIAS_GELU) {
#pragma unroll
    for (int k = 0; k < 4; ++k) {
      out[k] = pack_bf16x2(t[k]);
      out[4 + k] = pack_bf16x2(gelu2(unpack_bf16x2(out[k])));
    }
  } else if constexpr (EPI == MEMHIP_EPI_BIAS_GELU_DG) {
#pragma unroll
    for (int k = 0; k < 4; ++k) {
      ef32x2 g, dg;
      gelu_and_grad2(unpack_bf16x2(pack_bf16x2(t[k])), g, dg);
      out[k] = pack_f16x2(dg);
      out[4 + k] = pack_bf16x2(g);
    }
  } else if constexpr (EPI == MEMHIP_EPI_MUL_AUX) {
    const unsigned h[4] = {row.h.x, row.h.y, row.h.z, row.h.w};
#pragma unroll
    for (int k = 0; k < 4; ++k) out[k] = pack_bf16x2(unpack_bf16x2(pack_bf16x2(t[k])) * unpack_f16x2(h[k]));
    if (p.colsum) {
#pragma unroll
      for (int k = 0; k < 4; ++k) {
        const ef32x2 f = unpack_bf16x2(out[k]);
        cs[2 * k] += f.x;
        cs[2 * k + 1] += f.y;
      }
    }
  } else if constexpr (epi_resid(EPI)) {
    unsigned y[4];
    float x[8];
#pragma unroll
    for (int k = 0; k < 8; ++k) x[k] = row.x[k];
    float br[8];
#pragma unroll
    for (int k = 0; k < 4; ++k) {
      y[k] = pack_bf16x2(t[k]);
      const ef32x2 f = unpack_bf16x2(y[k]);
      br[2 * k] = f.x;
      br[2 * k + 1] = f.y;
    }
    if constexpr (EPI == MEMHIP_EPI_RESIDUAL_DROP) {
      const DropParams& d = drop_of(p);
      const unsigned kb = dropout_keep8(d, drop_row(p, row.row), (unsigned)(n >> 3));
#pragma unroll
      for (int k = 0; k < 8; ++k) br[k] = __fmul_rn(br[k], dropout_mul(d, kb, k));
    }
#pragma unroll
    for (int k = 0; k < 8; ++k) br[k] = __fmul_rn(c.g[k], br[k]);
    {
      const float rm = row.rm;
      const float kp = (p.rowmask || p.sample_map) ? p.keep_prob : 1.0f;
      const float rk = __frcp_rn(kp);
#pragma unroll
      for (int k = 0; k < 8; ++k) {
        const float q0 = br[k] * rk;
        const float q = fmaf(fmaf(-q0, kp, br[k]), rk, q0);
        br[k] = __fmul_rn(q, rm);
      }
    }
#pragma unroll
    for (int k = 0; k < 8; ++k) out[k] = __float_as_uint(__fadd_rn(x[k], br[k]));
    if constexpr (COPY == 1) st_branch_copy(p, m, n, y);
    if constexpr (COPY == 2)
      *(gu32x4_ptr)(reinterpret_cast<__bf16*>(p.out0) + (long long)m * p.ldo0 + n) = eu32x4{y[0], y[1], y[2], y[3]};
  } else if constexpr (EPI == MEMHIP_EPI_DGELU) {
    const unsigned h[4] = {row.h.x, row.h.y, row.h.z, row.h.w};
#pragma unroll
    for (int k = 0; k < 4; ++k) {
      const ef32x2 da = unpack_bf16x2(pack_bf16x2(t[k]));
      out[k] = pack_bf16x2(da * gelu_grad2(unpack_bf16x2(h[k])));
    }
    if (p.colsum) {
#pragma unroll
      for (int k = 0; k < 4; ++k) {
        const ef32x2 f = unpack_bf16x2(out[k]);
        cs[2 * k] += f.x;
        cs[2 * k + 1] += f.y;
      }
    }
  } else if constexpr (EPI == MEMHIP_EPI_F32) {
    float* o = reinterpret_cast<float*>(p.out0) + (long long)m * p.ldo0 + n;
    if (p.accumulate) {
      float x[8];
      ld8(o, x);
#pragma unroll
      for (int k = 0; k < 8; ++k) out[k] = __float_as_uint(x[k] + acc[k]);
    } else {
#pragma unroll
      for (int k = 0; k < 8; ++k) out[k] = __float_as_uint(acc[k]);
    }
  } else if constexpr (EPI == MEMHIP_EPI_PATCH_EMBED) {
    const float w = (float)reinterpret_cast<const unsigned char*>(p.aux)[m];
    float mt[8];
    ld8(p.vec1 + n, mt);
#pragma unroll
    for (int k = 0; k < 4; ++k) {
      const ef32x2 f = unpack_bf16x2(pack_bf16x2(t[k]));
      out[2 * k] = __float_as_uint(__fadd_rn(__fmul_rn(f.x, 1.0f - w), __fmul_rn(mt[2 * k], w)));
      out[2 * k + 1] = __float_as_uint(__fadd_rn(__fmul_rn(f.y, 1.0f - w), __fmul_rn(mt[2 * k + 1], w)));
    }
  }
}

template <int EPI>
__device__ __forceinline__ void epi8_store(const GemmArgs& p, int m, int n, long long rrow, const unsigned* out) {
  if constexpr (EPI == MEMHIP_EPI_BIAS_BF16 || EPI == MEMHIP_EPI_MUL_AUX || EPI == MEMHIP_EPI_DGELU) {
    st_stream16(p.out0, (long long)m * p.ldo0 + n, out[0], out[1], out[2], out[3]);
  } else if constexpr (EPI == MEMHIP_EPI_BIAS_GELU || EPI == MEMHIP_EPI_BIAS_GELU_DG) {
    st_stream16(p.out0, (long long)m * p.ldo0 + n, out[0], out[1], out[2], out[3]);
    st_stream16(p.out1, (long long)m * p.ldo1 + n, out[4], out[5], out[6], out[7]);
  } else {
    float x[8];
#pragma unroll
    for (int k = 0; k < 8; ++k) x[k] = __uint_as_float(out[k]);
    if constexpr (epi_resid(EPI)) {
      st8(p.resid + rrow * p.ldr + n, x);
    } else if constexpr (EPI == MEMHIP_EPI_F32) {
      st8(reinterpret_cast<float*>(p.out0) + (long long)m * p.ldo0 + n, x);
    } else if constexpr (EPI == MEMHIP_EPI_PATCH_EMBED) {
      const int L = p.rows_per_sample;
      const int b = m / L, pi = m - b * L;
      st8(p.resid + ((long long)b * (L + 1) + 1 + pi) * p.ldr + n, x);
    }
  }
}

template <int EPI, int COPY = 1>
__device__ __forceinline__ void epilogue8(const GemmArgs& p, int m, int n, const float* acc, float* cs, const EpiCols& c,
                                          const EpiRow<EPI>& row) {
  unsigned out[EpiPk<EPI>::W];
  epi8_math<EPI, COPY>(p, m, n, acc, cs, c, row, out);
  long long rrow = m;
  if constexpr (epi_resid(EPI)) rrow = row.row;
  epi8_store<EPI>(p, m, n, rrow, out);
}

__device__ __forceinline__ void epilogue8_residual_packed(const GemmArgs& p, int m, int n, const unsigned* y, const EpiCols& c,
                                                          const EpiRow<MEMHIP_EPI_RESIDUAL>& row) {
  float br[8], x[8];
#pragma unroll
  for (int k = 0; k < 4; ++k) {
    const ef32x2 f = unpack_bf16x2(y[k]);
    br[2 * k] = f.x;
    br[2 * k + 1] = f.y;
  }
  if (p.vec1) {
#pragma unroll
    for (int k = 0; k < 8; ++k) br[k] = __fmul_rn(c.g[k], br[k]);
  }
  if (p.rowmask || p.sample_map) {
    const float rm = row.rm;
    const float rk = __frcp_rn(p.keep_prob);
#pragma unroll
    for (int k = 0; k < 8; ++k) {
      const float q0 = br[k] * rk;
      const float q = fmaf(fmaf(-q0, p.keep_prob, br[k]), rk, q0);
      br[k] = __fmul_rn(q, rm);
    }
  }
#pragma unroll
  for (int k = 0; k < 8; ++k) x[k] = __fadd_rn(row.x[k], br[k]);
  st_branch_copy(p, m, n, y);
  st8(p.resid + row.row * p.ldr + n, x);
}

template <int EPI>
__device__ __forceinline__ void epilogue8(const GemmArgs& p, int m, int n, const float* acc, float* cs, const EpiCols& c) {
  EpiRow<EPI> row;
  epi_row_load<EPI>(p, m, n, row);
  epilogue8<EPI>(p, m, n, acc, cs, c, row);
}
template <int EPI>
__device__ __forceinline__ void epilogue8(const GemmArgs& p, int m, int n, const float* acc, float* cs) {
  EpiCols c;
  epi_cols_load<EPI>(p, n, c);
  epilogue8<EPI>(p, m, n, acc, cs, c);
}

__device__ __forceinline__ unsigned swap8(unsigned v) {
  return (unsigned)__builtin_amdgcn_update_dpp(0, (int)v, 0x128 , 0xf, 0xf, false);
}
__device__ __forceinline__ void pq_pack(const unsigned* a, const unsigned* b, bool hi, unsigned* P, unsigned* Q) {
#pragma unroll
  for (int k = 0; k < 4; ++k) {
    const unsigned sb = swap8(b[k]), sa = swap8(a[k]);
    P[k] = hi ? sb : a[k];
    Q[k] = hi ? b[k] : sa;
  }
}
__device__ __forceinline__ void pq_unpack(const unsigned* P, const unsigned* Q, bool hi, unsigned* a, unsigned* b) {
#pragma unroll
  for (int k = 0; k < 4; ++k) {
    const unsigned sq = swap8(Q[k]), sp = swap8(P[k]);
    a[k] = hi ? sq : P[k];
    b[k] = hi ? Q[k] : sp;
  }
}

template <int N>
__device__ __forceinline__ float dpp_row_shr(float v) {
  return __int_as_float(__builtin_amdgcn_update_dpp(0, __float_as_int(v), 0x110 + N, 0xf, 0xf, true));
}
__device__ __forceinline__ void colsum_flush16(const GemmArgs& p, int n, float* cs, int lane) {
  if (!p.colsum) return;
  float* const dst = colsum_base(p);
  float t[8];
#pragma unroll
  for (int k = 0; k < 8; ++k) {
    float v = cs[k];
    v += dpp_row_shr<1>(v);
    v += dpp_row_shr<2>(v);
    v += dpp_row_shr<4>(v);
    v += dpp_row_shr<8>(v);
    t[k] = v;
    cs[k] = 0.f;
  }
  if ((lane & 15) == 15) {
#pragma unroll
    for (int k = 0; k < 8; ++k) atomicAdd(dst + n + k, t[k]);
  }
}

__device__ __forceinline__ void colsum_flush(const GemmArgs& p, int n, float* cs, int lane) {
  if (!p.colsum) return;
  float* const dst = colsum_base(p);
#pragma unroll
  for (int k = 0; k < 8; ++k) {
    float v = cs[k];
    v += __shfl_xor(v, 8);
    v += __shfl_xor(v, 16);
// ... 12 lines not shown
```

mem_amd/csrc/gemm_nt_plan.hpp:

```cpp
#pragma once
#include "../../include/memhip.h"

namespace memhip {

struct GemmArgs {
  const __bf16* A; const __bf16* B;
  long long lda, ldb;
  int M, N, K, epilogue;
  void* out0; long long ldo0;
  void* out1; long long ldo1;
  const float* bias;
  const float* vec1;
  float* resid; long long ldr;
  const void* aux; long long ldaux;
  const float* rowmask;
  float keep_prob;
  float colscale; int colscale_n;
  int rows_per_sample;
  int accumulate;
  float* colsum;
  const int* sample_map;
  int colsum_copies;
  int reserved0;
  int m_base;
};

typedef memhip_nt_launch_t NtLaunch;
typedef memhip_nt_plan_t NtPlan;

struct NtOptions { int gemm_p8, gemm256, gemm_split, gemm_p8_half, gemm_p8_pair, gemm_p8_min_n, gemm256_min_n; };

inline bool nt_p8_copy(const GemmArgs& p) {
  return !(p.epilogue == MEMHIP_EPI_RESIDUAL_DROP || (p.epilogue == MEMHIP_EPI_RESIDUAL && !p.out0));
}
constexpr bool nt_p8_has(int epi, int bmt, bool guard, bool copy) {
  if (epi == MEMHIP_EPI_PATCH_EMBED || (bmt == 256 && guard)) return false;
  if (epi == MEMHIP_EPI_RESIDUAL_DROP) return bmt == 128 && !copy;
  if (epi == MEMHIP_EPI_RESIDUAL) return bmt == 128 || !copy;
  return copy;
}
constexpr bool nt_pair_has(int epi, bool copy) {
  return (epi == MEMHIP_EPI_BIAS_BF16 || epi == MEMHIP_EPI_RESIDUAL || epi == MEMHIP_EPI_BIAS_GELU_DG ||
          epi == MEMHIP_EPI_MUL_AUX) && copy == (epi != MEMHIP_EPI_RESIDUAL);
}
constexpr bool nt_g256_has(int epi) {
  return epi == MEMHIP_EPI_BIAS_BF16 || epi == MEMHIP_EPI_BIAS_GELU || epi == MEMHIP_EPI_RESIDUAL ||
         epi == MEMHIP_EPI_RESIDUAL_DROP || epi == MEMHIP_EPI_DGELU || epi == MEMHIP_EPI_F32;
}

NtPlan gemm_nt_plan(const GemmArgs& p, int stream_cus, int device_cus, const NtOptions& o);

}
```

mem_amd/ops.py:

```python
import ctypes as C

import torch

from ._lib import check, declare, f32, f64, i32, i64, lib, ptr, stream_ptr, sz, vp
from .vae_model import pack_convt_weight

EPI_BIAS_BF16, EPI_BIAS_GELU, EPI_RESIDUAL, EPI_DGELU, EPI_F32, EPI_PATCH_EMBED, EPI_BIAS_GELU_DG, EPI_MUL_AUX = range(8)
EPI_RESIDUAL_DROP = 8


class Dropout(C.Structure):
    _fields_ = [("key0", C.c_uint32), ("key1", C.c_uint32), ("site", C.c_uint32), ("thr", C.c_uint32), ("scale", f32),
                ("row0", i32)]


def dropout_params(key0, key1, site, p, row0=0):
    assert 0.0 <= p < 1.0, p
    return Dropout(int(key0) & 0xFFFFFFFF, int(key1) & 0xFFFFFFFF, int(site), int(round(p * 65536)), 1.0 / (1.0 - p), int(row0))


def with_row0(d, row0):
    return None if d is None else Dropout(d.key0, d.key1, d.site, d.thr, d.scale, int(row0))


class GemmArgs(C.Structure):
    _fields_ = [("A", vp), ("B", vp), ("lda", i64), ("ldb", i64),
                ("M", i32), ("N", i32), ("K", i32), ("epilogue", i32),
                ("out0", vp), ("ldo0", i64), ("out1", vp), ("ldo1", i64),
                ("bias", vp), ("vec1", vp), ("resid", vp), ("ldr", i64),
                ("aux", vp), ("ldaux", i64), ("rowmask", vp), ("keep_prob", f32),
                ("colscale", f32), ("colscale_n", i32), ("rows_per_sample", i32), ("accumulate", i32),
                ("colsum", vp), ("sample_map", vp), ("colsum_copies", i32), ("reserved0", i32),
                ("dropout", vp)]


class Branch(C.Structure):
    _fields_ = [("y", vp), ("ldy", i64), ("gamma", vp), ("rowmask", vp), ("keep_prob", f32), ("rows_per_sample", i32),
                ("dy", vp), ("lddy", i64), ("dgamma", vp), ("dbias", vp), ("out_map", vp), ("dropout", vp)]


class BranchBwdArgs(C.Structure):
    _fields_ = [("dx", vp), ("lddx", i64), ("M", i32), ("D", i32), ("branch", Branch)]


class LnBwdBranchArgs(C.Structure):
    _fields_ = [("dy", vp), ("lddy", i64), ("x", vp), ("ldx", i64), ("R", i32), ("D", i32), ("gamma", vp), ("mean", vp),
                ("rstd", vp), ("dres", vp), ("lddres", i64), ("dgamma", vp), ("dbeta", vp), ("in_map", vp), ("branch", Branch)]


class AttnBwdArgs(C.Structure):
    _fields_ = [("qkv", vp), ("ldqkv", i64), ("dout", vp), ("ldo", i64), ("out", vp), ("ldout", i64), ("lse", vp), ("delta", vp),
                ("table", vp), ("window_h", i32), ("window_w", i32), ("B", i32), ("T", i32), ("D", i32), ("heads", i32),
                ("scale", f32), ("reserved0", i32), ("dqkv", vp), ("lddqkv", i64), ("dtable", vp), ("dq_bias", vp),
                ("dv_bias", vp), ("ws", vp), ("ws_bytes", i64)]


class NtLaunch(C.Structure):
    _fields_ = [(n, i32) for n in ("kind", "row0", "rows", "tail_rows", "guard", "copy", "grid", "tail_grid")]


class NtPlan(C.Structure):
    _fields_ = [("count", i32), ("l", NtLaunch * 2)]


declare({"memhip_gemm_bf16_nt": (i32, [C.POINTER(GemmArgs), vp]),
         "memhip_branch_bwd": (i32, [C.POINTER(BranchBwdArgs), vp]),
         "memhip_layernorm_bwd_branch": (i32, [C.POINTER(LnBwdBranchArgs), vp]),
         "memhip_attn_bwd": (i32, [C.POINTER(AttnBwdArgs), vp]),
         "memhip_gemm_bf16_nt_plan": (i32, [C.POINTER(GemmArgs), i32, i32, C.POINTER(NtPlan)])})


def _p(t):
    return None if t is None else t.data_ptr()


GEMM_TIMER = None
GEMM_EVENT_POOL = []


def _timer_event():
    return GEMM_EVENT_POOL.pop() if GEMM_EVENT_POOL else torch.cuda.Event(enable_timing=True)


def _timed(code, flops, fn):
    if GEMM_TIMER is None:
        fn()
        return
    e0, e1 = _timer_event(), _timer_event()
    e0.record()
    fn()
    e1.record()
    GEMM_TIMER.append((e0, e1, flops, code))


def gemm_args(A, B, M, N, K, epi, out0=None, out1=None, bias=None, vec1=None, resid=None, aux=None,
              rowmask=None, keep_prob=1.0, colscale=1.0, colscale_n=0, rows_per_sample=1, accumulate=False, colsum=None,
              lda=None, ldb=None, ldo0=None, ldo1=None, ldr=None, ldaux=None, sample_map=None, colsum_copies=0, dropout=None):
    a = GemmArgs()
    a.A, a.B = _p(A), _p(B)
    a.lda = A.stride(0) if lda is None else lda
    a.ldb = B.stride(0) if ldb is None else ldb
    a.M, a.N, a.K, a.epilogue = M, N, K, epi
    a.out0 = _p(out0)
    a.ldo0 = (out0.stride(0) if out0 is not None else 0) if ldo0 is None else ldo0
    a.out1 = _p(out1)
    a.ldo1 = (out1.stride(0) if out1 is not None else 0) if ldo1 is None else ldo1
    a.bias, a.vec1, a.resid = _p(bias), _p(vec1), _p(resid)
    a.ldr = (resid.stride(0) if resid is not None else 0) if ldr is None else ldr
    a.aux = _p(aux)
    a.ldaux = (aux.stride(0) if (aux is not None and aux.dim() > 1) else 0) if ldaux is None else ldaux
    a.rowmask = _p(rowmask)
    a.keep_prob, a.colscale, a.colscale_n = keep_prob, colscale, colscale_n
    a.rows_per_sample, a.accumulate = rows_per_sample, int(accumulate)
    a.colsum = _p(colsum)
    a.sample_map = _p(sample_map)
    a.colsum_copies = colsum_copies
    a.dropout = None if dropout is None else C.addressof(dropout)
    return a


def gemm_nt(A, B, M, N, K, epi, *args, **kw):
    a = gemm_args(A, B, M, N, K, epi, *args, **kw)
    _timed(epi, 2.0 * M * N * K, lambda: check(lib.memhip_gemm_bf16_nt(C.byref(a), stream_ptr()), "gemm_bf16_nt"))


NT_128, NT_G256, NT_P8_256, NT_P8_128, NT_P8_PAIR = range(5)


def gemm_nt_plan(a, stream_cus=None, device_cus=None):
    if stream_cus is None or device_cus is None:
        cus = torch.cuda.get_device_properties(torch.cuda.current_device()).multi_processor_count
        stream_cus = cus if stream_cus is None else stream_cus
        device_cus = cus if device_cus is None else device_cus
    plan = NtPlan()
    check(lib.memhip_gemm_bf16_nt_plan(C.byref(a), stream_cus, device_cus, C.byref(plan)), "gemm_bf16_nt_plan")
    return [plan.l[i] for i in range(plan.count)]


declare({
    "memhip_layernorm_fwd": (i32, [vp, i64, vp, i32, i32, vp, vp, f32, vp, i64, vp, vp, vp]),
    "memhip_layernorm_bwd": (i32, [vp, i64, vp, i64, vp, i32, i32, vp, vp, vp, vp, i64, i32, vp, vp, vp]),
    "memhip_layerscale_grad": (i32, [vp, i64, vp, i64, vp, vp, vp, i32, i32, vp, vp]),
    "memhip_embed_bwd": (i32, [vp, i64, vp, i32, i32, i32, vp, i64, vp, vp, vp]),
    "memhip_cross_entropy": (i32, [vp, i64, vp, i32, i32, f32, vp, vp, i32, vp, vp]),
    "memhip_attn_tokens_padded": (i32, [i32]),
    "memhip_relpos_gather": (i32, [vp, vp, i32, i32, i32, vp, vp, vp]),
    "memhip_attn_fwd": (i32, [vp, i64, i32, i32, i32, i32, vp, i32, i32, vp, i64, vp, vp]),
    "memhip_attn_delta": (i32, [vp, vp, i64, i64, i32, vp, vp]),
    "memhip_attn_bwd_workspace": (i64, [i32, i32, i32, i32, i32]),
    "memhip_cast_f32_bf16": (i32, [vp, vp, i64, vp]),
    "memhip_copy_samples_f32": (i32, [vp, vp, vp, i32, i64, vp]),
    "memhip_zero": (i32, [vp, i64, vp]),
    "memhip_stream_reserve_cus": (i32, [vp, i32]),
    "memhip_zero_ranges": (i32, [vp, vp, i32, i64, vp]),
    "memhip_transpose_cast_f32_bf16": (i32, [vp, i64, i32, i32, vp, i64, vp]),
    "memhip_transpose_bf16": (i32, [vp, i64, i32, i32, vp, i64, i32, vp, i32, i32, vp, i32, i32, vp]),
    "memhip_im2col_bf16": (i32, [vp, i32, i32, i32, i32, i32, i32, vp, vp]),
    "memhip_fill_cls": (i32, [vp, i64, i32, i32, i32, vp, vp]),
    "memhip_gemv_bf16_acc": (i32, [vp, i64, i32, i32, vp, vp, vp, vp, vp]),
    "memhip_nchw_to_padded_nhwc4": (i32, [vp, i32, i32, i32, i32, vp, vp, vp, i64, i32, vp]),
    "memhip_argmax_rows": (i32, [vp, i32, i64, i32, i32, vp, vp, vp, vp, i32, vp]),
    "memhip_tok_flag_samples": (i32, [vp, vp, i32, i32, f32, vp, vp, vp, vp]),
    "memhip_tok_gather_images_f32": (i32, [vp, i32, i32, i32, vp, vp, vp, vp, i32, i32, vp, vp, vp]),
    "memhip_tok_scatter_ids": (i32, [vp, vp, vp, i32, i32, i32, vp, vp]),
    "memhip_grad_norm_workspace": (sz, []),
    "memhip_grad_norm": (i32, [vp, i64, vp, vp, sz, vp]),
    "memhip_adamw": (i32, [vp, vp, vp, vp, i64, vp, f64, f64, f64, f64, f64, i32, vp, f64, vp]),
    "memhip_transpose_cast_batched": (i32, [vp, vp, i32, i32, vp]),
    "memhip_adamw_groups": (i32, [vp, vp, vp, vp, i64, vp, vp, i32, f64, f64, f64, i32, vp, f64, vp]),
    "memhip_dropout_mask": (i32, [C.POINTER(Dropout), i32, i32, i32, vp, vp]),
    "memhip_dropout_rows_f32": (i32, [C.POINTER(Dropout), vp, i64, i32, i32, vp]),
})


def dropout_mask(d, row0, rows, cols, out):
    check(lib.memhip_dropout_mask(C.byref(d), row0, rows, cols, ptr(out), stream_ptr()), "dropout_mask")


def dropout_rows(d, x, rows, D):
    check(lib.memhip_dropout_rows_f32(C.byref(d), ptr(x), x.stride(0), rows, D, stream_ptr()), "dropout_rows_f32")


def layernorm_fwd(x, gamma, beta, y, mean, rstd, R, D, eps=1e-6, row_idx=None):
    check(lib.memhip_layernorm_fwd(ptr(x), x.stride(0), ptr(row_idx), R, D, ptr(gamma), ptr(beta), eps,
                                   ptr(y), y.stride(0), ptr(mean), ptr(rstd), stream_ptr()), "layernorm_fwd")


def layernorm_bwd(dy, x, gamma, mean, rstd, dres, dgamma, dbeta, R, D, accumulate=True, row_idx=None):
    check(lib.memhip_layernorm_bwd(ptr(dy), dy.stride(0), ptr(x), x.stride(0), ptr(row_idx), R, D, ptr(gamma),
                                   ptr(mean), ptr(rstd), ptr(dres), dres.stride(0), int(accumulate),
                                   ptr(dgamma), ptr(dbeta), stream_ptr()), "layernorm_bwd")


def _branch(y, gamma, rowmask, keep_prob, rows_per_sample, dy, dgamma, dbias, out_map, dropout):
    return Branch(_p(y), y.stride(0) if y is not None else 0, _p(gamma), _p(rowmask), keep_prob, rows_per_sample, _p(dy),
                  dy.stride(0), _p(dgamma), _p(dbias), _p(out_map), None if dropout is None else C.addressof(dropout))


def layernorm_bwd_branch(dy, x, gamma, mean, rstd, dres, dgamma, dbeta, R, D, y_b, gamma_b, dy_b, dgamma_b, dbias_b,
                         rowmask=None, keep_prob=1.0, rows_per_sample=1, in_map=None, out_map=None, dropout=None):
    a = LnBwdBranchArgs(_p(dy), dy.stride(0), _p(x), x.stride(0), R, D, _p(gamma), _p(mean), _p(rstd), _p(dres), dres.stride(0),
                        _p(dgamma), _p(dbeta), _p(in_map),
                        _branch(y_b, gamma_b, rowmask, keep_prob, rows_per_sample, dy_b, dgamma_b, dbias_b, out_map, dropout))
    check(lib.memhip_layernorm_bwd_branch(C.byref(a), stream_ptr()), "layernorm_bwd_branch")


def layerscale_grad(W16, dW, bias, dbias, gamma, N, K, dgamma):
    check(lib.memhip_layerscale_grad(ptr(W16), W16.stride(0), ptr(dW), dW.stride(0), ptr(bias), ptr(dbias), ptr(gamma),
                                     N, K, ptr(dgamma), stream_ptr()), "layerscale_grad")


def branch_bwd(dx, y, gamma, dy, dgamma, dbias, M, D, rowmask=None, keep_prob=1.0, rows_per_sample=1, out_map=None, dropout=None):
    a = BranchBwdArgs(_p(dx), dx.stride(0), M, D,
                      _branch(y, gamma, rowmask, keep_prob, rows_per_sample, dy, dgamma, dbias, out_map, dropout))
    check(lib.memhip_branch_bwd(C.byref(a), stream_ptr()), "branch_bwd")


def gemv_acc(W, N, K, x, y, x_acc=None, zero=None):
    check(lib.memhip_gemv_bf16_acc(ptr(W), W.stride(0), N, K, ptr(x), ptr(y), ptr(x_acc), ptr(zero), stream_ptr()),
          "gemv_bf16_acc")


CONV_MODES = ("bf16", "fp32", "fp16x2")
_CONV_MODE = {torch.bfloat16: 0, torch.float32: 1, torch.float16: 2}
_F16X2 = 2


class ConvArgs(C.Structure):
    _fields_ = [("mode", i32), ("reserved0", i32), ("in", vp), ("in_plane", i64), ("weight", vp), ("w_plane", i64),
                ("bias", vp), ("add", vp), ("add_plane", i64), ("out", vp), ("out_plane", i64)] + \
               [(n, i32) for n in ("B", "H", "W", "Cin", "Cout", "ksize", "stride", "pad", "relu", "out_padded", "out_f32",
                                   "reserved1")] + [("n_active", vp)]


declare({"memhip_conv2d_nhwc": (i32, [C.POINTER(ConvArgs), vp])})


def conv_args(mode, B, H, W, Cin, Cout, ksize, stride, pad, x=None, weight=None, bias=None, out=None, relu=False, add=None,
              out_padded=True, out_f32=False, n_active=None, planes=(0, 0, 0, 0)):
    return ConvArgs(mode, 0, x, planes[0], weight, planes[1], bias, add, planes[2], out, planes[3], B, H, W, Cin, Cout, ksize,
                    stride, pad, int(relu), int(out_padded), int(out_f32), 0, n_active)


def conv2d_nhwc(x_pad, weight, bias, out, B, H, W, Cin, Cout, ksize, stride, pad, relu=False, add=None, out_padded=True,
                n_active=None):
    mode = _CONV_MODE[x_pad.dtype]
    out_f32 = mode == _F16X2 and out.dtype == torch.float32
    assert weight.dtype == x_pad.dtype and (out_f32 or out.dtype == x_pad.dtype) and (add is None or add.dtype == x_pad.dtype)
    planes = (0, 0, 0, 0) if mode != _F16X2 else (x_pad.stride(0), weight.stride(0), 0 if add is None else add.stride(0),
                                             0 if out_f32 else out.stride(0))
    a = conv_args(mode, B, H, W, Cin, Cout, ksize, stride, pad, _p(x_pad), _p(weight), _p(bias), _p(out), relu, _p(add),
                  out_padded and not out_f32, out_f32, _p(n_active), planes)
    check(lib.memhip_conv2d_nhwc(C.byref(a), stream_ptr()), "conv2d_nhwc")


def nchw_to_padded_nhwc4(x, out, mean=None, std=None):
    B, Cc, H, W = x.shape
    mode = _CONV_MODE[out.dtype]
    check(lib.memhip_nchw_to_padded_nhwc4(ptr(x), B, Cc, H, W, ptr(mean), ptr(std), ptr(out), out.stride(0) if mode == _F16X2 else 0,
                                          mode, stream_ptr()), "nchw_to_padded_nhwc4")


def argmax_rows(logits, M, N, ids, gap=None, rms=None, n_samples=None, rows_per_sample=0):
    check(lib.memhip_argmax_rows(ptr(logits), _CONV_MODE[logits.dtype], logits.stride(0), M, N, ptr(ids), ptr(gap), ptr(rms),
                                 ptr(n_samples), rows_per_sample, stream_ptr()), "argmax_rows")


declare({
    "memhip_convt2d_nhwc": (i32, [vp, vp, vp, vp, i32, i32, i32, i32, i32, i32, vp]),
    "memhip_kl_uniform_rows": (i32, [vp, i32, i64, i32, i32, vp, vp]),
})


def convt2d_nhwc(x_pad, weight, bias, out, B, H, W, Cin, Cout, relu=False):
    assert x_pad.dtype == torch.bfloat16 and weight.dtype == torch.bfloat16 and out.dtype == torch.bfloat16
    assert B == 0 or (x_pad.numel() >= B * (H + 2) * (W + 2) * Cin and weight.numel() == 16 * Cin * Cout and
                      out.numel() >= B * (2 * H + 2) * (2 * W + 2) * Cout and (bias is None or bias.numel() == Cout))
    check(lib.memhip_convt2d_nhwc(_p(x_pad), _p(weight), _p(bias), _p(out), B, H, W, Cin, Cout, int(relu), stream_ptr()),
          "convt2d_nhwc")


def kl_uniform_rows(logits, M, N, out=None):
    assert logits.dim() == 2 and logits.stride(1) == 1 and logits.shape[0] >= M and logits.shape[1] >= N
    if out is None:
        out = torch.empty((M,), dtype=torch.float32, device=logits.device)
    assert out.dtype == torch.float32 and out.numel() >= M
    check(lib.memhip_kl_uniform_rows(ptr(logits), _CONV_MODE[logits.dtype], logits.stride(0), M, N, ptr(out), stream_ptr()),
          "kl_uniform_rows")
    return out[:M]


def tok_flag_samples(gap, rms, B, hw, kappa, lst, count, stats=None):
    check(lib.memhip_tok_flag_samples(ptr(gap), ptr(rms), B, hw, float(kappa), ptr(lst), ptr(count), ptr(stats), stream_ptr()),
          "tok_flag_samples")


def tok_gather_images(x, mean, std, lst, count, offset, R, out, n_round):
    _, Cc, H, W = x.shape
    check(lib.memhip_tok_gather_images_f32(ptr(x), Cc, H, W, ptr(mean), ptr(std), ptr(lst), ptr(count), offset, R, ptr(out),
                                           ptr(n_round), stream_ptr()), "tok_gather_images_f32")


def tok_scatter_ids(ids_in, lst, n_round, offset, R, hw, ids_out):
    check(lib.memhip_tok_scatter_ids(ptr(ids_in), ptr(lst), ptr(n_round), offset, R, hw, ptr(ids_out), stream_ptr()),
          "tok_scatter_ids")


def embed_bwd(dx, mask_u8, B, L, D, dy, dcls, dmask_token):
    check(lib.memhip_embed_bwd(ptr(dx), dx.stride(0), ptr(mask_u8), B, L, D, ptr(dy), dy.stride(0), ptr(dcls),
                               ptr(dmask_token), stream_ptr()), "embed_bwd")


def cross_entropy(logits, labels, M, V, grad_scale, row_loss, row_correct, out2, write_grad=True):
    check(lib.memhip_cross_entropy(ptr(logits), logits.stride(0), ptr(labels), M, V, grad_scale, ptr(row_loss),
                                   ptr(row_correct), int(write_grad), ptr(out2), stream_ptr()), "cross_entropy")


def attn_tokens_padded(T):
    return lib.memhip_attn_tokens_padded(T)


def relpos_gather(table, index_i32, T, TP, heads, bias_pad, biasT_pad=None):
    check(lib.memhip_relpos_gather(ptr(table), ptr(index_i32), T, TP, heads, ptr(bias_pad), ptr(biasT_pad),
                                   stream_ptr()), "relpos_gather")


def attn_fwd(qkv, B, T, D, heads, table, window, out, lse):
    _timed(200, 4.0 * B * T * T * D, lambda: check(
        lib.memhip_attn_fwd(ptr(qkv), qkv.stride(0), B, T, D, heads, ptr(table), window[0], window[1], ptr(out),
                            out.stride(0), ptr(lse), stream_ptr()), "attn_fwd"))


def attn_delta(dout, out, rows, heads, delta):
    check(lib.memhip_attn_delta(ptr(dout), ptr(out), out.stride(0), rows, heads, ptr(delta), stream_ptr()),
          "attn_delta")


def attn_bwd_workspace(B, T, heads, window):
    return int(lib.memhip_attn_bwd_workspace(B, T, heads, window[0], window[1]))


ATTN_16, ATTN_SMALL, ATTN_WIN, ATTN_WIN_DS, ATTN_STREAM = range(1, 6)
ATTN_KERNELS = ("attn_stats_zero_kernel", "attn_delta_kernel", "attn_fwd_kernel", "attn_bwd_kv_kernel", "attn_bwd_q_kernel",
                "attn16_fwd_kernel", "attn16_bwd_kernel", "attn_win_stats_kernel", "attn_fwd_win_kernel", "attn_bwd_kv_win_kernel",
                "attn_bwd_q_win_kernel", "attn_bwd_kvs_win_kernel", "attn_bwd_qs_win_kernel", "attn_fwd_stream_kernel",
                "attn_bwd_kv_stream_kernel", "attn_bwd_q_stream_kernel")


class AttnLaunch(C.Structure):
    _fields_ = [(n, i32) for n in ("kernel", "grid_x", "grid_y", "grid_z", "block", "lds")]


class AttnPlan(C.Structure):
    _fields_ = [(n, i32) for n in ("family", "n", "ww", "vb", "dt", "fd", "spb", "nwg", "groups", "nbz", "nbq", "nbs", "qgroups",
                                   "qs", "stream_spb", "lds_over", "count")] + [("l", AttnLaunch * 5)]

    @property
    def launches(self):
        return [(ATTN_KERNELS[l.kernel], (l.grid_x, l.grid_y, l.grid_z), l.block, l.lds) for l in self.l[:self.count]]


declare({"memhip_attn_plan_fwd": (i32, [i32, i32, i32, i32, i32, i32, i32, C.POINTER(AttnPlan)]),
         "memhip_attn_plan_bwd": (i32, [i32, i32, i32, i32, i32, i32, i32, i32, i32, vp, i64, i32, C.POINTER(AttnPlan)])})


def attn_plan(B, T, heads, window, backward=False, dtable=True, dv_bias=False, out=False, ws=None, ws_bytes=0, stream_cus=None):
    if stream_cus is None:
        stream_cus = torch.cuda.get_device_properties(torch.cuda.current_device()).multi_processor_count
    plan = AttnPlan()
    if not backward:
        check(lib.memhip_attn_plan_fwd(B, T, 64 * heads, heads, window[0], window[1], stream_cus, C.byref(plan)), "attn_plan_fwd")
        return plan
    if ws is not None and not isinstance(ws, int):
        ws, ws_bytes = ptr(ws), ws.numel() * ws.element_size()
    check(lib.memhip_attn_plan_bwd(B, T, 64 * heads, heads, window[0], window[1], int(dtable), int(dv_bias), int(out), ws, ws_bytes,
# ... 967 lines not shown
```

mem_amd/vit_engine.py:

```python
import math
from collections import namedtuple

import torch

from . import ops

ALIGN = 1024

Branch = namedtuple("Branch", "n rows gemm_rows ridx smap cmap rowmask keep_prob")


def _pad(n, a):
    return (n + a - 1) // a * a


def flat_layout(shapes, skip, order, aliases=()):
    decays = lambda n: not (len(shapes[n]) == 1 or n.endswith(".bias") or n in skip)
    segs, buckets, flags, off = {}, [], [], 0
    for bname, entries in order:
        b0 = off
        for e in entries:
            if isinstance(e, tuple):
                (n, k), flag = e, 0
            elif e in shapes:
                n, k, flag = e, math.prod(shapes[e]), int(decays(e))
            else:
                continue
            segs[n] = (off, k)
            size = _pad(k, ALIGN)
            flags += [flag] * (size // ALIGN)
            off += size
        buckets.append((bname, b0, off))
    for alias, seg, o, k in aliases:
        segs[alias] = (segs[seg][0] + o, k)
    missing = [n for n in shapes if n not in segs]
    assert not missing, f"parameters not placed in the flat buffer: {missing}"
    return segs, buckets, off, flags, [n for n in shapes if decays(n)]


def check_export(export, depth, what="export"):
    if export is None:
        return ()
    export = tuple(int(i) for i in export)
    for k, i in enumerate(export):
        if not 0 <= i < depth:
            raise ValueError(f"{what}: block index {i} outside [0, {depth})")
        if i in export[:k]:
            raise ValueError(f"{what}: block index {i} given twice")
        if k and i < export[k - 1]:
            raise ValueError(f"{what}: block indices must ascend, {i} follows {export[k - 1]}")
    return export


class FlatParams:

    def _pack_flat(self, named, skip, order, aliases=()):
        self.segs, self.buckets, self.nflat, flags, self.decay_names = flat_layout(
            {n: tuple(p.shape) for n, p in named.items()}, skip, order, aliases)
        self.flat_p = torch.zeros(self.nflat, dtype=torch.float32, device=self.dev)
        self.flat_g = torch.zeros(self.nflat, dtype=torch.float32, device=self.dev)
        self.wd_flags = torch.tensor(flags, dtype=torch.uint8, device=self.dev)
        self.named = named
        for n, p in named.items():
            o, k = self.segs[n]
            view = self.flat_p[o:o + k].view(p.shape)
            view.copy_(p.data)
            p.data = view
        self.attach_grads()

    def attach_grads(self):
        for n, p in self.named.items():
            o, k = self.segs[n]
            g = p.grad
            if g is None or g.data_ptr() != self.flat_g.data_ptr() + 4 * o:
                p.grad = self.flat_g[o:o + k].view(p.shape)

    def P(self, name):
        o, k = self.segs[name]
        return self.flat_p[o:o + k]

    def G(self, name):
        o, k = self.segs[name]
        return self.flat_g[o:o + k]


class ViTEngine(FlatParams):
    def __init__(self, model):
        self.model = model
        p0 = next(model.parameters())
        assert p0.is_cuda, "mem_amd runs on the GPU only: move the model to cuda first (no CPU fallback)"
        self.dev = p0.device
        pe = model.patch_embed
        self.C = pe.proj.weight.shape[1]
        self.ph, self.pw = pe.patch_size
        self.H, self.W = pe.img_size
        self.L = pe.num_patches
        self.T = self.L + 1
        self.D = model.embed_dim
        self.depth = len(model.blocks)
        self.heads = model.blocks[0].attn.num_heads
        self.scale = float(model.blocks[0].attn.scale)
        self.hidden = model.blocks[0].mlp.fc1.weight.shape[0]
        self.head_kind = "mlm" if hasattr(model, "lm_head") else "cls"
        self.V = model.lm_head.weight.shape[0] if self.head_kind == "mlm" else 0
        self.Kpe = self.C * self.ph * self.pw
        assert self.D % 64 == 0 and self.hidden % 64 == 0 and self.Kpe % 64 == 0, "GEMM K dims must be multiples of 64"
        self.has_pos = model.pos_embed is not None
        self.drop_rate = float(getattr(model, "drop_rate", 0.0))
        self.window = tuple(pe.patch_shape)
        self.nrd = (2 * self.window[0] - 1) * (2 * self.window[1] - 1) + 3
        if model.rel_pos_bias is not None:
            self.rel = "shared"
        elif getattr(model.blocks[0].attn, "relative_position_bias_table", None) is not None:
            self.rel = "block"
        else:
            self.rel = "none"
        self.TP = ops.attn_tokens_padded(self.T)
        self._pack_parameters()
        self._build_static()
        if hasattr(model, "register_state_dict_pre_hook"):
            model.register_state_dict_pre_hook(lambda *_a, **_k: self.wait_optimizer())
        self.B = 0
        self.Mm_cap = 0
        self.cur = None
        self.B_stash = 0
        self.step_masks = None
        self.weights_dirty = True
        self.w16_version = 0
        self._zero_plans = {}
        self.grad_hook = None
        self.hook_on_side = True
        self.accumulate_grads = False
        self.overlap_optimizer = False
        self._opt_stream = None
        self._opt_ev = None
        self._opt_done = None
        self.wgrad_side_stream = True
        self.wgrad_group = 2
        self.fwd_two_streams = False
        self._side = None
        self._ev_pool, self._ev_i = [], 0
        self.dp_skip = True
        self.tail_rows = True
        self._dp_stage = None

    def _pack_parameters(self):
        m, D = self.model, self.D
        order, aliases = [], []
        head = ["lm_head.weight", "lm_head.bias", "head.weight", "head.bias", "fc_norm.weight", "fc_norm.bias", "norm.weight",
                "norm.bias"]
        head += [n for n, _ in m.named_parameters() if n.startswith(tuple(getattr(m, "_TAIL_PREFIXES", ()))) and n not in head]
        order.append(("head", head))
        for i in reversed(range(self.depth)):
            pre = f"blocks.{i}."
            qkvb = pre + "attn.qkvbias3"
            aliases += [(pre + "attn.q_bias", qkvb, 0, D), (pre + "attn.v_bias", qkvb, 2 * D, D)]
            names = [pre + n for n in ("mlp.fc2.weight", "mlp.fc2.bias", "gamma_2", "mlp.fc1.weight", "mlp.fc1.bias",
                                       "norm2.weight", "norm2.bias", "attn.proj.weight", "attn.proj.bias", "gamma_1",
                                       "attn.qkv.weight")]
            names += [(qkvb, 3 * D)] + [pre + n for n in ("attn.relative_position_bias_table", "norm1.weight", "norm1.bias")]
            order.append((f"block{i}", names))
        order.append(("embed", ["rel_pos_bias.relative_position_bias_table", "patch_embed.proj.weight",
                                "patch_embed.proj.bias", "mask_token", "cls_token", "pos_embed"]))
        self._pack_flat(dict(m.named_parameters()), m.no_weight_decay(), order, aliases)
        self.flat_w16 = torch.zeros(self.nflat, dtype=torch.bfloat16, device=self.dev)
        self.no_decay_names = [n for n in self.named if n not in set(self.decay_names)]

    def W16(self, name, rows, cols):
        o, k = self.segs[name]
        return self.flat_w16[o:o + k].view(rows, cols)

    def _build_static(self):
        D, Hd, V, dev = self.D, self.hidden, self.V, self.dev
        bf = torch.bfloat16
        self.wT = {}
        for i in range(self.depth):
            self.wT[i] = dict(qkv=torch.empty((D, 3 * D), dtype=bf, device=dev),
                              proj=torch.empty((D, D), dtype=bf, device=dev),
                              fc1=torch.empty((D, Hd), dtype=bf, device=dev),
                              fc2=torch.empty((Hd, D), dtype=bf, device=dev))
        self.wT_lm = torch.empty((D, V), dtype=bf, device=dev) if self.head_kind == "mlm" else None
        self.zero_table = torch.zeros((self.nrd, self.heads), dtype=torch.float32, device=dev)
        self.zero_vec = torch.zeros(D, dtype=torch.float32, device=dev)
        self.head_end = self.buckets[0][2]
        self._tdesc = None
        self.set_gelu_dg(True)
        self.fuse_ln_branch = True
        self.gn_ws = torch.zeros(1024, dtype=torch.float64, device=dev)
        self.gnorm = torch.zeros(1, dtype=torch.float32, device=dev)
        self.loss_acc = torch.zeros(2, dtype=torch.float32, device=dev)

    def _matrix_grad_names(self):
        names = [f"blocks.{i}.{n}" for i in range(self.depth) for n in ("attn.qkv.weight", "attn.proj.weight", "mlp.fc1.weight",
                                                                       "mlp.fc2.weight")]
        names.append("patch_embed.proj.weight")
        if self.head_kind == "mlm":
            names.append("lm_head.weight")
        return names

    def _zero_small_grads(self, start=0):
        key = ("zr", start)
        if key not in self._zero_plans:
            import numpy as np
            mats = sorted(self.segs[n] for n in self._matrix_grad_names())
            ranges, pos = [], start
            for o, k in mats:
                end = o + _pad(k, ALIGN)
                if end <= start:
                    continue
                if o > pos:
                    ranges.append((pos * 4, (o - pos) * 4))
                pos = max(pos, end)
            if pos < self.nflat:
                ranges.append((pos * 4, (self.nflat - pos) * 4))
            arr = np.asarray(ranges, dtype=np.int64).reshape(-1, 2)
            self._zero_plans[key] = (torch.from_numpy(arr).to(self.dev), len(ranges), int(arr[:, 1].sum()) if len(ranges) else 0)
        dev, n, total = self._zero_plans[key]
        ops.zero_ranges(self.flat_g, dev, n, total)

    def _zero_grad_of(self, name):
        o, k = self.segs[name]
        ops.zero_(self.flat_g[o:o + _pad(k, ALIGN)])

    def set_gelu_dg(self, on):
        self.epi_gelu, self.epi_dgelu = (ops.EPI_BIAS_GELU_DG, ops.EPI_MUL_AUX) if on else (ops.EPI_BIAS_GELU, ops.EPI_DGELU)

    def ensure_batch(self, B, Mm_max, keep=True):
        if B > self.B:
            self._alloc_forward(B)
        if keep and self.B_stash < self.B:
            self._alloc_stash()
        if Mm_max > self.Mm_cap or (self.head_kind == "mlm" and not hasattr(self, "hN")):
            self._alloc_head(min(self.B * self.L, _pad(Mm_max + Mm_max // 16 + 1, 256)))

    def _alloc_head(self, Mm_cap):
        dev, bf, f32 = self.dev, torch.bfloat16, torch.float32
        D, V = self.D, self.V
        e = lambda *s, dt=bf: torch.empty(s, dtype=dt, device=dev)
        if self.head_kind == "mlm":
            self.hN = e(Mm_cap, D)
            self.meanN, self.rstdN = e(Mm_cap, dt=f32), e(Mm_cap, dt=f32)
            self.logits = e(Mm_cap, V)
            self.row_loss, self.row_ok = e(Mm_cap, dt=f32), torch.empty(Mm_cap, dtype=torch.int32, device=dev)
            self.dhN = e(Mm_cap, D)
            self.x_tail, self.dxc = e(max(Mm_cap, 1), D, dt=f32), e(max(Mm_cap, 1), D, dt=f32)
            self.y_tail = torch.zeros((_pad(max(Mm_cap, 1), 256), D), dtype=bf, device=dev)
        self.Mm_cap = Mm_cap

    def _act_set(self, B):
        dev, bf, f32 = self.dev, torch.bfloat16, torch.float32
        D, Hd, M = self.D, self.hidden, B * self.T
        Ma = M + 256
        e = lambda *s, dt=bf: torch.empty(s, dtype=dt, device=dev)
        z = lambda *s, dt=bf: torch.zeros(s, dtype=dt, device=dev)
        return dict(h1=z(Ma, D), qkv=z(Ma, 3 * D), ao=z(Ma, D), h2=z(Ma, D), hpre=z(Ma, Hd),
                    a=z(Ma, Hd), lse=e(B, self.heads, self.TP, dt=f32),
                    mean1=e(M, dt=f32), rstd1=e(M, dt=f32), mean2=e(M, dt=f32), rstd2=e(M, dt=f32))

    def _alloc_forward(self, B):
        dev, f32 = self.dev, torch.float32
        D, T = self.D, self.T
        M = B * T
        self.patches = torch.empty((B * self.L, self.Kpe), dtype=torch.bfloat16, device=dev)
        self.x = [torch.zeros((M + T, D), dtype=f32, device=dev) for _ in range(3)]
        self.act = [self._act_set(B)]
        if self.head_kind != "mlm":
            self.zero_mask = torch.zeros(B * self.L, dtype=torch.uint8, device=dev)
        for name in ("dx", "dY", "dh_small", "dY2", "dbig", "dqkv", "dao", "delta_ws", "_tn_ws", "bias_scr", "cs_ws", "dYpe"):
            if hasattr(self, name):
                delattr(self, name)
        self._maps = []
        self.B, self.B_stash = B, 0

    def _map_buffers(self, n, B):
        D, L = self.D, self.L
        while len(self._maps) < n:
            self._maps.append(torch.empty(self.B * D * L, dtype=torch.float32, device=self.dev))
        return [m[: B * D * L].view(B, D, *self.window) for m in self._maps[:n]]

    def _alloc_stash(self):
        dev, bf, f32 = self.dev, torch.bfloat16, torch.float32
        D, Hd, T, B = self.D, self.hidden, self.T, self.B
        M = B * T
        Ma = M + 256
        e = lambda *s, dt=bf: torch.empty(s, dtype=dt, device=dev)
        z = lambda *s, dt=bf: torch.zeros(s, dtype=dt, device=dev)
        self.x += [torch.zeros((M + T, D), dtype=f32, device=dev) for _ in range(2 * self.depth + 1 - len(self.x))]
        self.act += [self._act_set(B) for _ in range(self.depth - len(self.act))]
        self.dx = torch.zeros((M, D), dtype=f32, device=dev)
        self.dY, self.dh_small = z(Ma, D), z(Ma, D)
        self.dY2 = z(Ma, D)
        self.dbig = z(Ma, Hd)
        self.dqkv = z(Ma, 3 * D)
        self.dao = z(Ma, D)
        self.delta_ws = e(2 * M + 4, self.heads, dt=f32)
        self._tn_ws = torch.empty(0, dtype=torch.uint8, device=dev)
        self.bias_scr = torch.zeros(2, D, dtype=f32, device=dev)
        self.cs_ws = torch.zeros(self.CS_COPIES, self.hidden, dtype=f32, device=dev)
        self.dYpe = e(B * self.L, D)
        self.B_stash = B

    def sync_weights(self):
        self.wait_optimizer()
        ops.cast_f32_bf16(self.flat_p, self.flat_w16, self.nflat)
        if self._tdesc is None:
            self._build_transpose_descs()
        ops.transpose_cast_batched(self._tdesc, self._tprefix, self._tn, self._ttiles)
        self.weights_dirty = False
        self.w16_version += 1

    def _build_transpose_descs(self):
        import numpy as np
        D, Hd = self.D, self.hidden
        items = []
        for i in range(self.depth):
            pre = f"blocks.{i}."
            items += [(self.P(pre + "attn.qkv.weight"), 3 * D, D, self.wT[i]["qkv"]),
                      (self.P(pre + "attn.proj.weight"), D, D, self.wT[i]["proj"]),
                      (self.P(pre + "mlp.fc1.weight"), Hd, D, self.wT[i]["fc1"]),
                      (self.P(pre + "mlp.fc2.weight"), D, Hd, self.wT[i]["fc2"])]
        if self.head_kind == "mlm":
            items.append((self.P("lm_head.weight"), self.V, D, self.wT_lm))
        desc = np.zeros((len(items), 6), dtype=np.int64)
        prefix = np.zeros(len(items) + 1, dtype=np.int32)
        for k, (src, R, Cc, dst) in enumerate(items):
            desc[k] = (src.data_ptr(), Cc, R, Cc, dst.data_ptr(), dst.stride(0))
            prefix[k + 1] = prefix[k] + ((R + 63) // 64) * ((Cc + 63) // 64)
        self._tdesc = torch.from_numpy(desc).to(self.dev)
        self._tprefix = torch.from_numpy(prefix).to(self.dev)
        self._tn, self._ttiles = len(items), int(prefix[-1])
        self._tbucket = {}
        locs = []
        for i in range(self.depth):
            locs.append((f"block{i}", 4 * i, 4))
        if self.head_kind == "mlm":
            locs.append(("head", 4 * self.depth, 1))
        loc_prefix = []
        for name, k0, n in locs:
            pl = (prefix[k0:k0 + n + 1] - prefix[k0]).astype(np.int32)
            self._tbucket[name] = (k0, n, len(loc_prefix), int(pl[-1]))
            loc_prefix += list(pl)
        self._tprefix_loc = torch.from_numpy(np.asarray(loc_prefix, dtype=np.int32)).to(self.dev)

    def table(self, i):
        if self.rel == "shared":
            return self.P("rel_pos_bias.relative_position_bias_table")
        if self.rel == "block":
            return self.P(f"blocks.{i}.attn.relative_position_bias_table")
        return self.zero_table

    def dtable(self, i):
        if self.rel == "shared":
            return self.G("rel_pos_bias.relative_position_bias_table")
        if self.rel == "block":
            return self.G(f"blocks.{i}.attn.relative_position_bias_table")
        return None

    CS_COPIES = 8

    def _dp_plan(self, dp_masks, B):
        import numpy as np
        if dp_masks is None or not self.dp_skip:
            return None
        probs = [float(b.drop_prob) for b in self.model.blocks for _ in range(2)]
        if max(probs) == 0.0:
            return None
        mk = dp_masks.detach().cpu().numpy() if isinstance(dp_masks, torch.Tensor) else np.asarray(dp_masks)
        mk = mk.reshape(2 * self.depth, B) != 0
        J, T = 2 * self.depth, self.T
        W = 3 * B + 256
        host = np.zeros((J, W), dtype=np.int32)
        host[:, B + 256:2 * B + 256] = -1
        kept_n = []
        for j in range(J):
            if probs[j] == 0.0:
                kept_n.append(None)
                continue
            k = np.flatnonzero(mk[j]).astype(np.int32)
            d = np.flatnonzero(~mk[j]).astype(np.int32)
            host[j, :len(k)] = k
            host[j, len(k):B + 256] = B
            host[j, B + 256 + k] = np.arange(len(k), dtype=np.int32)
            host[j, 2 * B + 256:2 * B + 256 + len(d)] = d
            kept_n.append(len(k))
        if self._dp_stage is None or self._dp_stage_w != J * W:
            from .utils import HostStager
            self._dp_stage, self._dp_stage_w = HostStager(J * W * 4, self.dev), J * W
            self._dp_ar = torch.arange(T, dtype=torch.int32, device=self.dev)
        dev = self._dp_stage.put(host).view(torch.int32).view(J, W)
        ridx = (dev[:, :B, None] * T + self._dp_ar[None, None, :]).view(J, B * T)
        return dict(n=kept_n, kidx=dev[:, :B + 256], cmap=dev[:, B + 256:2 * B + 256], drop=dev[:, 2 * B + 256:], ridx=ridx, B=B)

    def _branches(self, B, plan, dp_masks):
        T, out = self.T, []
        for j in range(2 * self.depth):
            drop_prob = self.model.blocks[j // 2].drop_prob
            if plan is not None and plan["n"][j] is not None:
                n = plan["n"][j]
                out.append(Branch(n, n * T, _pad(n * T, 256), plan["ridx"][j], plan["kidx"][j], plan["cmap"][j], None,
                                  1.0 - drop_prob))
            else:
                rowmask = dp_masks[j] if (dp_masks is not None and drop_prob > 0.0) else None
                out.append(Branch(B, B * T, B * T, None, None, None, rowmask, 1.0 - drop_prob))
        return out

    def _drop(self, site, row0=0):
        key = self.cur["drop_key"] if self.cur else None
        if key is None:
            return None
        return ops.dropout_params(key[0], key[1], site, self.drop_rate, row0)

    def _copy_dropped(self, plan, j, src, dst, B):
        nd = B - plan["n"][j]
        if nd > 0:
            ops.copy_samples(src, dst, plan["drop"][j], nd, self.T * self.D)

    def forward(self, x, mask_u8, rows_idx, labels=None, dp_masks=None, all_tokens=False, labels_event=None):
        assert x.is_cuda and x.dtype == torch.float32 and x.is_contiguous()
        B = x.shape[0]
        assert tuple(x.shape[1:]) == (self.C, self.H, self.W), \
            f"Input image size ({x.shape[2]}*{x.shape[3]}) doesn't match model ({self.H}*{self.W})."
        Mm = rows_idx.numel()
        self.ensure_batch(B, Mm)
        use_tail = (self.tail_rows and not all_tokens and self.depth >= 1 and 0 < Mm and 4 * Mm <= 3 * B * self.T)
        xl = self.forward_trunk(x, mask_u8, dp_masks, tail_rows=rows_idx if use_tail else None)
        D, Hd, T, L, V = self.D, self.hidden, self.T, self.L, self.V
        M = B * T
        self.cur.update(Mm=Mm, rows=rows_idx, labels=labels)
        self._wait_params("head")
        if self.cur.get("tail") is not None:
            ops.layernorm_fwd(self.x_tail, self.P("norm.weight"), self.P("norm.bias"), self.hN, self.meanN, self.rstdN, Mm, D)
        else:
            ops.layernorm_fwd(xl, self.P("norm.weight"), self.P("norm.bias"), self.hN, self.meanN, self.rstdN, Mm, D,
                              row_idx=rows_idx)
        ops.gemm_nt(self.hN, self.W16("lm_head.weight", V, D), Mm, V, D, ops.EPI_BIAS_BF16, out0=self.logits,
                    bias=self.P("lm_head.bias"))
        if labels is not None:
            if labels_event is not None:
                torch.cuda.current_stream().wait_event(labels_event)
            ops.cross_entropy(self.logits, labels, Mm, V, 1.0 / Mm, self.row_loss, self.row_ok, self.loss_acc,
                              write_grad=True)
        return self.logits[:Mm]

    def _split_point(self, B, num_cu=256):
        ntn = max(1, self.D // 256)
        tile_rows = -(-B * self.T // 256)
        rounds = tile_rows * ntn // num_cu
        if rounds < 1:
            return 0
        bs = (rounds * num_cu // ntn) * 256 // self.T
        return bs if 0 < bs < B and (B - bs) * self.T >= 4096 else 0
# ... 18 lines not shown
        g1 = self.P(pre + "gamma_1") if (pre + "gamma_1") in self.segs else None
        g2 = self.P(pre + "gamma_2") if (pre + "gamma_2") in self.segs else None
        tail = self.cur["tail"] if (i == self.depth - 1 and b0 == 0 and b1 == B) else None
        if ba.smap is not None:
            self._copy_dropped(plan, 2 * i, xin, xmid, B)
        if ba.n > 0:
            rs = slice(r0, r1) if ba.smap is None else slice(None)
            h1, qkv, ao = a["h1"][rs], a["qkv"][rs], a["ao"][rs]
            ops.layernorm_fwd(xin, self.P(pre + "norm1.weight"), self.P(pre + "norm1.bias"), h1, a["mean1"][r0:r1],
                              a["rstd1"][r0:r1], ba.rows, D, row_idx=ba.ridx)
            ops.gemm_nt(h1, self.W16(pre + "attn.qkv.weight", 3 * D, D), ba.gemm_rows, 3 * D, D, ops.EPI_BIAS_BF16,
                        out0=qkv, bias=self.P(pre + "attn.qkvbias3"), colscale=self.scale, colscale_n=D)
            ops.attn_fwd(qkv, ba.n, T, D, self.heads, self.table(i), self.window, ao, a["lse"][b0:b1])
            da = self._drop(2 * i, r0)
            ops.gemm_nt(ao, self.W16(pre + "attn.proj.weight", D, D), ba.gemm_rows, D, D,
                        ops.EPI_RESIDUAL if da is None else ops.EPI_RESIDUAL_DROP, out0=None,
                        bias=self.P(pre + "attn.proj.bias"), vec1=g1, resid=xmid, aux=xin, ldaux=D, rowmask=ba.rowmask,
                        keep_prob=ba.keep_prob, rows_per_sample=T, sample_map=ba.smap, dropout=da)
        if tail is not None:
            self._mlp_fwd_tail(i, a, xs[2 * i + 1], g2, bm.keep_prob, tail)
            return
        if bm.smap is not None:
            self._copy_dropped(plan, 2 * i + 1, xmid, xout, B)
        if bm.n > 0:
            rs = slice(r0, r1) if bm.smap is None else slice(None)
            h2, hpre, aa = a["h2"][rs], a["hpre"][rs], a["a"][rs]
            ops.layernorm_fwd(xmid, self.P(pre + "norm2.weight"), self.P(pre + "norm2.bias"), h2, a["mean2"][r0:r1],
                              a["rstd2"][r0:r1], bm.rows, D, row_idx=bm.ridx)
            ops.gemm_nt(h2, self.W16(pre + "mlp.fc1.weight", Hd, D), bm.gemm_rows, Hd, D, self.epi_gelu, out0=hpre,
                        out1=aa, bias=self.P(pre + "mlp.fc1.bias"))
            dm = self._drop(2 * i + 1, r0)
            ops.gemm_nt(aa, self.W16(pre + "mlp.fc2.weight", D, Hd), bm.gemm_rows, D, Hd,
                        ops.EPI_RESIDUAL if dm is None else ops.EPI_RESIDUAL_DROP, out0=None,
                        bias=self.P(pre + "mlp.fc2.bias"), vec1=g2, resid=xout, aux=xmid, ldaux=D, rowmask=bm.rowmask,
                        keep_prob=bm.keep_prob, rows_per_sample=T, sample_map=bm.smap, dropout=dm)

    def _mlp_fwd_tail(self, i, a, xmid, g2, keep, tail):
        D, Hd = self.D, self.hidden
        pre = f"blocks.{i}."
        rows, Mm = tail["rows"], tail["Mm"]
        Mp = _pad(Mm, 256)
        assert self._drop(0) is None, "the tail-row form of the last block is pretraining-only: no element-wise dropout"
        ops.layernorm_fwd(xmid, self.P(pre + "norm2.weight"), self.P(pre + "norm2.bias"), a["h2"], a["mean2"], a["rstd2"],
                          Mm, D, row_idx=rows)
        ops.gemm_nt(a["h2"], self.W16(pre + "mlp.fc1.weight", Hd, D), Mp, Hd, D, self.epi_gelu, out0=a["hpre"],
                    out1=a["a"], bias=self.P(pre + "mlp.fc1.bias"))
        ops.gemm_nt(a["a"], self.W16(pre + "mlp.fc2.weight", D, Hd), Mp, D, Hd, ops.EPI_BIAS_BF16, out0=self.y_tail,
                    bias=self.P(pre + "mlp.fc2.bias"))
        ops.residual_rows(xmid, rows, self.y_tail, g2, tail["rowkeep"], keep, Mm, D, self.x_tail)

    def forward_trunk(self, x, mask_u8=None, dp_masks=None, tail_rows=None, drop_key=None, keep=True, export=None,
                      streams=None):
        export = check_export(export, self.depth)
        assert (not export and streams is None) or (self.head_kind == "cls" and tail_rows is None), \
            "per-block exports serve the finetuning trunk: no mlm head, no tail-row form"
        assert drop_key is None or (self.drop_rate > 0.0 and tail_rows is None), "dropout: finetuning trunk only"
        assert keep or (self.head_kind == "cls" and tail_rows is None), \
            "forward-only mode (keep=False) serves the finetuning trunk: no mlm head, no tail-row form"
        assert x.is_cuda and x.dtype == torch.float32 and x.is_contiguous()
        B = x.shape[0]
        assert tuple(x.shape[1:]) == (self.C, self.H, self.W), \
            f"Input image size ({x.shape[2]}*{x.shape[3]}) doesn't match model ({self.H}*{self.W})."
        self.ensure_batch(B, self.Mm_cap, keep=keep)
        if self.weights_dirty:
            self.sync_weights()
        if self.fwd_two_streams:
            self.wait_optimizer()
        self._wait_params("embed")
        if mask_u8 is None:
            mask_u8 = self.zero_mask[: B * self.L]
        D, Hd, T, L = self.D, self.hidden, self.T, self.L
        M = B * T
        plan = self._dp_plan(dp_masks, B)
        if plan is not None:
            dp_masks = None
        nx = 2 * self.depth + 1
        self.cur = dict(B=B, M=M, Mm=0, mask=mask_u8, rows=None, dp=dp_masks, labels=None, plan=plan, tail=None, drop_key=drop_key,
                        keep=bool(keep), x=self.x if keep else [self.x[j % 3] for j in range(nx)],
                        act=self.act if keep else [self.act[0]] * self.depth, branch=self._branches(B, plan, dp_masks),
                        maps=dict(zip(export, self._map_buffers(len(export), B))) if export else None, streams=streams, dmaps=None)
        if tail_rows is not None and not self.fwd_two_streams:
            jm, lastb = 2 * self.depth - 1, self.model.blocks[self.depth - 1]
            keepvec = None
            if lastb.drop_prob > 0.0:
                if plan is not None and plan["n"][jm] is not None:
                    keepvec = (plan["cmap"][jm] >= 0).to(torch.float32)
                elif dp_masks is not None:
                    keepvec = dp_masks[jm]
            rowkeep = None
            if keepvec is not None:
                rowkeep = keepvec.index_select(0, torch.div(tail_rows, T, rounding_mode="floor").long()).contiguous()
            self.cur["tail"] = dict(rows=tail_rows, Mm=tail_rows.numel(), rowkeep=rowkeep)
        if self.head_kind == "cls" and not self.accumulate_grads and self.head_end:
            ops.zero_(self.flat_g[: self.head_end])
        ops.im2col(x, B, self.C, self.H, self.W, self.ph, self.pw, self.patches)
        x0 = self.x[0]
        if not keep and plan is not None:
            ops.zero_(x0[M:M + T])
        ops.fill_cls(x0, B, T, D, self.P("cls_token"))
        ops.gemm_nt(self.patches, self.W16("patch_embed.proj.weight", D, self.Kpe), B * L, D, self.Kpe,
                    ops.EPI_PATCH_EMBED, bias=self.P("patch_embed.proj.bias"),
                    vec1=self.P("mask_token") if "mask_token" in self.segs else self.zero_vec,
                    resid=x0, aux=mask_u8, rows_per_sample=L, ldaux=0)
        if self.has_pos:
            x0[:M].view(B, T, D).add_(self.P("pos_embed").view(1, T, D))
        dpos = self._drop(2 * self.depth)
        if dpos is not None:
            ops.dropout_rows(dpos, x0, M, D)
        bs = self._split_point(B) if (self.fwd_two_streams and ops.GEMM_TIMER is None and plan is None) else 0
        split = 0 < bs < B
        if split:
            if self._side is None:
                self._side = torch.cuda.Stream(device=self.dev)
            e0 = torch.cuda.Event()
            e0.record()
            self._side.wait_event(e0)
            for i in range(self.depth):
                self._block_fwd(i, 0, bs)
                self._export_block(i, 0, bs)
                with torch.cuda.stream(self._side):
                    self._block_fwd(i, bs, B)
                    self._export_block(i, bs, B)
            e1 = torch.cuda.Event()
            e1.record(self._side)
            torch.cuda.current_stream().wait_event(e1)
        else:
            for i in range(self.depth):
                self._wait_params(f"block{i}")
                self._block_fwd(i, 0, B)
                self._export_block(i, 0, B)
        return self.cur["x"][2 * self.depth][:M]

    def _export_block(self, i, b0, b1):
        c = self.cur
        if c["maps"] is None and c["streams"] is None:
            return
        xout, T = c["x"][2 * i + 2], self.T
        if c["maps"] is not None and i in c["maps"]:
            ops.tokens_to_maps(xout, c["B"], T, out=c["maps"][i], b0=b0, b1=b1)
        if c["streams"] is not None:
            c["streams"][i][b0 * T:b1 * T].copy_(xout[b0 * T:b1 * T])

    def _tn_ws_at_least(self, need):
        if need > self._tn_ws.numel():
            self._tn_ws = torch.empty(need, dtype=torch.uint8, device=self.dev)

    def _wgrad(self, dY, X, R, n_out, n_in, gname, bias_grads=()):
        self._tn_ws_at_least(ops.gemm_tn_workspace(R, n_out, n_in))
        ops.gemm_tn(dY, X, R, n_out, n_in, self.G(gname).view(n_out, n_in), accumulate=self.accumulate_grads,
                    workspace=self._tn_ws)
        for gv, c0, c1 in bias_grads:
            ops.colsum_bf16(dY[:, c0:c1], R, c1 - c0, gv)

    def _wg_mlp(self, pre, a, has_g, R, dY):
        D, Hd = self.D, self.hidden
        both = int(self.wgrad_group) >= 2
        if both:
            self._wgrad_group([(dY, a["a"], R, D, Hd, pre + "mlp.fc2.weight"), (self.dbig, a["h2"], R, Hd, D, pre + "mlp.fc1.weight")])
        else:
            self._wgrad(dY, a["a"], R, D, Hd, pre + "mlp.fc2.weight")
        self._side_read_done("dY")
        if has_g:
            ops.layerscale_grad(self.W16(pre + "mlp.fc2.weight", D, Hd), self.G(pre + "mlp.fc2.weight").view(D, Hd),
                                self.P(pre + "mlp.fc2.bias"), self.G(pre + "mlp.fc2.bias"),
                                self.P(pre + "gamma_2"), D, Hd, self.G(pre + "gamma_2"))
        if not both:
            self._wgrad(self.dbig, a["h2"], R, Hd, D, pre + "mlp.fc1.weight")
        self._side_read_done("dbig")

    def _wgrad_group(self, items):
        self._tn_ws_at_least(ops.gemm_tn_group_workspace([(R, n_out, n_in) for _, _, R, n_out, n_in, _ in items]))
        ops.gemm_tn_group([(dY, X, R, n_out, n_in, self.G(gname).view(n_out, n_in)) for dY, X, R, n_out, n_in, gname in items],
                          accumulate=self.accumulate_grads, workspace=self._tn_ws)

    def _event(self):
        if self._ev_i == len(self._ev_pool):
            self._ev_pool.append(torch.cuda.Event())
        e = self._ev_pool[self._ev_i]
        self._ev_i += 1
        return e

    def _side_begin(self):
        self._use_side = bool(self.wgrad_side_stream) and ops.GEMM_TIMER is None
        self._ev_i = 0
        self._side_reads = {}
        if self._use_side and self._side is None:
            self._side = torch.cuda.Stream(device=self.dev)
        if self._use_side and getattr(self, "_ws_for", None) != (self.B, self.Mm_cap):
            self._ws_for = (self.B, self.Mm_cap)
            D, Hd = self.D, self.hidden
            M = self.B * self.T
            self._tn_ws_at_least(max(
                ops.gemm_tn_group_workspace([(M, D, D), (M, 3 * D, D)]), ops.gemm_tn_group_workspace([(M, D, Hd), (M, Hd, D)]),
                ops.gemm_tn_workspace(M, 3 * D, D), ops.gemm_tn_workspace(M, Hd, D), ops.gemm_tn_workspace(M, D, Hd),
                ops.gemm_tn_workspace(M, D, D), ops.gemm_tn_workspace(self.Mm_cap or M, max(self.V, 1), D),
                ops.gemm_tn_workspace(self.B * self.L, D, self.Kpe)))

    def _on_side(self, fn):
        if not self._use_side:
            fn()
            return
        e = self._event()
        e.record()
        with torch.cuda.stream(self._side):
            self._side.wait_event(e)
            fn()

    def _side_read_done(self, name):
        if self._use_side:
            e = self._event()
            e.record(self._side)
            self._side_reads[name] = e

    def _before_overwrite(self, name):
        if self._use_side:
            e = self._side_reads.pop(name, None)
            if e is not None:
                torch.cuda.current_stream().wait_event(e)

    def _side_join(self):
        if not self._use_side:
            return
        e = self._event()
        e.record(self._side)
        torch.cuda.current_stream().wait_event(e)

    def _bucket_ready(self, k):
        if not self.grad_hook:
            return
        if not self._use_side:
            self.grad_hook(k)
            return
        if not self.hook_on_side:
            self._side_join()
            self.grad_hook(k)
            return
        e = self._event()
        e.record()
        with torch.cuda.stream(self._side):
            self._side.wait_event(e)
            self.grad_hook(k)

    attn_ds_workspace = True

    def _attn_ws(self, nb):
        if not self.attn_ds_workspace:
            return None
        need = ops.attn_bwd_workspace(nb, self.T, self.heads, self.window)
        if need == 0:
            return None
        ws = getattr(self, "_attn_ws_buf", None)
        if ws is None or ws.numel() < need:
            ws = self._attn_ws_buf = torch.empty(ops.attn_bwd_workspace(self.cur["B"], self.T, self.heads, self.window),
                                                 dtype=torch.uint8, device=self.dev)
        return ws

    def backward(self, dlogits=None):
        c = self.cur
        B, M, Mm = c["B"], c["M"], c["Mm"]
        D, Hd, T, L, V = self.D, self.hidden, self.T, self.L, self.V
        dp_masks = c["dp"]
        self.wait_optimizer()
        if dlogits is not None:
            self.logits[:Mm].copy_(dlogits)
        if not self.accumulate_grads:
            self._zero_small_grads()
        dx = self.dx
        ops.zero_(dx[:M])
        dl = self.logits
        self._side_begin()
        ops.gemm_nt(dl, self.wT_lm, Mm, D, V, ops.EPI_BIAS_BF16, out0=self.dhN)
        self._on_side(lambda: self._wgrad(dl, self.hN, Mm, V, D, "lm_head.weight", bias_grads=((self.G("lm_head.bias"), 0, V),)))
        if c.get("tail") is not None:
            ops.layernorm_bwd(self.dhN, self.x_tail, self.P("norm.weight"), self.meanN, self.rstdN, self.dxc,
                              self.G("norm.weight"), self.G("norm.bias"), Mm, D, accumulate=False)
            ops.scatter_rows(self.dxc, c["rows"], Mm, D, dx)
        else:
            ops.layernorm_bwd(self.dhN, self.x[2 * self.depth], self.P("norm.weight"), self.meanN, self.rstdN, dx,
                              self.G("norm.weight"), self.G("norm.bias"), Mm, D, accumulate=False, row_idx=c["rows"])
        self._backward_trunk()

    def backward_trunk(self, dxl, dmaps=None):
        c = self.cur
        if not c.get("keep", True):
            raise RuntimeError("backward_trunk after forward_trunk(keep=False): a forward-only pass keeps no activations "
                               "(the blocks shared one buffer set); run the forward with keep=True to train the trunk")
        M, D = c["M"], self.D
        if not self.accumulate_grads:
            self._zero_small_grads(self.head_end)
        if dxl is None:
            ops.zero_(self.dx[:M])
        else:
            self.dx[:M].copy_(dxl.reshape(M, D))
        if dmaps is not None:
            B, n = c["B"], c["B"] * D * self.L
            for i, g in dmaps.items():
                if not 0 <= i < self.depth:
                    raise ValueError(f"dmaps: block index {i} outside [0, {self.depth})")
                assert g.is_cuda and g.dtype == torch.float32 and g.is_contiguous() and g.numel() == n, \
                    f"dmaps[{i}]: contiguous fp32 [{B}, {D}, {self.window[0]}, {self.window[1]}]"
        c["dmaps"] = dmaps or None
        self._side_begin()
        self._backward_trunk()

    def _inject_dmap(self, i):
        dm = self.cur.get("dmaps")
        if dm is not None and i in dm:
            ops.maps_to_tokens_add(dm[i], self.dx, self.cur["B"], self.T)

    def _attn_branch_bwd(self, i, scr):
        pre = f"blocks.{i}."
        ba = self.cur["branch"][2 * i]
        self._before_overwrite("dY2")
        ops.branch_bwd(self.dx, None, self.P(pre + "gamma_1") if (pre + "gamma_1") in self.segs else None, self.dY2, None, scr,
                       self.cur["M"], self.D, rowmask=ba.rowmask, keep_prob=ba.keep_prob, rows_per_sample=self.T,
                       out_map=ba.cmap, dropout=self._drop(2 * i))

    def _mlp_bwd_tail(self, i, a, pre, has_g, keep, tail, scr):
        D, Hd = self.D, self.hidden
        rows, Mm, rk = tail["rows"], tail["Mm"], tail["rowkeep"]
        Mp = _pad(Mm, 256)
        assert self._drop(0) is None, "the tail-row form of the last block is pretraining-only: no element-wise dropout"
        dx, dY = self.dx, self.dY
        self._before_overwrite("dY")
        ops.branch_bwd(self.dxc, None, self.P(pre + "gamma_2") if has_g else None, dY, None, self.G(pre + "mlp.fc2.bias"),
                       Mm, D, rowmask=rk, keep_prob=keep, rows_per_sample=1)
        if Mp > Mm:
            ops.zero_(dY[Mm:Mp])
        self._before_overwrite("dbig")
        ops.gemm_nt(dY, self.wT[i]["fc2"], Mp, Hd, D, self.epi_dgelu, out0=self.dbig, aux=a["hpre"],
                    colsum=self.cs_ws, colsum_copies=self.CS_COPIES)
        ops.colsum_fold(self.cs_ws, self.CS_COPIES, Hd, self.G(pre + "mlp.fc1.bias"))
        self._on_side(lambda: self._wg_mlp(pre, a, has_g, Mm, dY))
        ops.gemm_nt(self.dbig, self.wT[i]["fc1"], Mp, D, Hd, ops.EPI_BIAS_BF16, out0=self.dh_small)
        ops.layernorm_bwd(self.dh_small, self.x[2 * i + 1], self.P(pre + "norm2.weight"), a["mean2"], a["rstd2"], dx,
                          self.G(pre + "norm2.weight"), self.G(pre + "norm2.bias"), Mm, D, accumulate=True, row_idx=rows)
        self._attn_branch_bwd(i, scr)

    def _backward_trunk(self):
        c = self.cur
        B, M, br = c["B"], c["M"], c["branch"]
        D, Hd, T = self.D, self.hidden, self.T
        dx, dY, dY2 = self.dx, self.dY, self.dY2
        self._bucket_ready(0)
        ops.zero_(self.bias_scr)
        fuse = D <= 1024 and self.fuse_ln_branch
        self._inject_dmap(self.depth - 1)
        for i in reversed(range(self.depth)):
            pre = f"blocks.{i}."
            a = self.act[i]
            ba, bm = br[2 * i], br[2 * i + 1]
            xin, xmid = self.x[2 * i], self.x[2 * i + 1]
            has_g = (pre + "gamma_1") in self.segs
            table, dtable = self.table(i), self.dtable(i)
            scr = self.bias_scr[i & 1]
            tail = c["tail"] if i == self.depth - 1 else None
            if tail is not None:
                self._mlp_bwd_tail(i, a, pre, has_g, bm.keep_prob, tail, scr)
            else:
                if i == self.depth - 1 or not fuse:
                    self._before_overwrite("dY")
                    ops.branch_bwd(dx, None, self.P(pre + "gamma_2") if has_g else None, dY, None, self.G(pre + "mlp.fc2.bias"),
                                   M, D, rowmask=bm.rowmask, keep_prob=bm.keep_prob, rows_per_sample=T, out_map=bm.cmap,
                                   dropout=self._drop(2 * i + 1))
                if bm.n == 0 and not self.accumulate_grads:
                    self._zero_grad_of(pre + "mlp.fc1.weight")
                    self._zero_grad_of(pre + "mlp.fc2.weight")
                if bm.n > 0:
                    self._before_overwrite("dbig")
                    if bm.gemm_rows > bm.rows:
                        ops.zero_(dY[bm.rows:bm.gemm_rows])
                    ops.gemm_nt(dY, self.wT[i]["fc2"], bm.gemm_rows, Hd, D, self.epi_dgelu, out0=self.dbig, aux=a["hpre"],
                                colsum=self.cs_ws, colsum_copies=self.CS_COPIES)
                    ops.colsum_fold(self.cs_ws, self.CS_COPIES, Hd, self.G(pre + "mlp.fc1.bias"))
                    self._on_side(lambda: self._wg_mlp(pre, a, has_g, bm.rows, dY))
                    ops.gemm_nt(self.dbig, self.wT[i]["fc1"], bm.gemm_rows, D, Hd, ops.EPI_BIAS_BF16, out0=self.dh_small)
                if fuse:
                    self._before_overwrite("dY2")
                    ops.layernorm_bwd_branch(self.dh_small, xmid, self.P(pre + "norm2.weight"), a["mean2"], a["rstd2"], dx,
                                             self.G(pre + "norm2.weight"), self.G(pre + "norm2.bias"), M, D, None,
                                             self.P(pre + "gamma_1") if has_g else None, dY2, None, scr,
                                             rowmask=ba.rowmask, keep_prob=ba.keep_prob, rows_per_sample=T,
                                             in_map=bm.cmap, out_map=ba.cmap, dropout=self._drop(2 * i))
                else:
                    if bm.n > 0:
                        ops.layernorm_bwd(self.dh_small, xmid, self.P(pre + "norm2.weight"), a["mean2"], a["rstd2"], dx,
                                          self.G(pre + "norm2.weight"), self.G(pre + "norm2.bias"), bm.rows, D, accumulate=True,
                                          row_idx=bm.ridx)
                    self._attn_branch_bwd(i, scr)
            if ba.n == 0 and not self.accumulate_grads:
                self._zero_grad_of(pre + "attn.proj.weight")
                self._zero_grad_of(pre + "attn.qkv.weight")
            if ba.n > 0:
                ops.gemm_nt(dY2, self.wT[i]["proj"], ba.gemm_rows, D, D, ops.EPI_BIAS_BF16, out0=self.dao)
            ops.gemv_acc(self.wT[i]["proj"], D, D, scr, self.G(pre + "attn.v_bias"),
                         x_acc=self.G(pre + "attn.proj.bias"), zero=self.bias_scr[(i & 1) ^ 1])
            if ba.n > 0:
                def wg_proj(grouped=False):
                    if not grouped:
                        self._wgrad(dY2, a["ao"], ba.rows, D, D, pre + "attn.proj.weight")
                    self._side_read_done("dY2")
                    if has_g:
                        ops.layerscale_grad(self.W16(pre + "attn.proj.weight", D, D), self.G(pre + "attn.proj.weight").view(D, D),
                                            self.P(pre + "attn.proj.bias"), self.G(pre + "attn.proj.bias"),
                                            self.P(pre + "gamma_1"), D, D, self.G(pre + "gamma_1"))
                if not self.wgrad_group:
                    self._on_side(wg_proj)
                self._before_overwrite("dqkv")
                ops.attn_bwd(a["qkv"], self.dao, a["lse"], self.delta_ws, table, self.window, ba.n, T, D, self.heads,
                             self.scale, self.dqkv, dtable, dq_bias=self.G(pre + "attn.q_bias"), out=a["ao"],
                             ws=self._attn_ws(ba.n))

                def wg_qkv():
                    if self.wgrad_group:
                        self._wgrad_group([(dY2, a["ao"], ba.rows, D, D, pre + "attn.proj.weight"),
                                           (self.dqkv, a["h1"], ba.rows, 3 * D, D, pre + "attn.qkv.weight")])
                        wg_proj(grouped=True)
                    else:
                        self._wgrad(self.dqkv, a["h1"], ba.rows, 3 * D, D, pre + "attn.qkv.weight")
                    self._side_read_done("dqkv")
                self._on_side(wg_qkv)
                ops.gemm_nt(self.dqkv, self.wT[i]["qkv"], ba.gemm_rows, D, 3 * D, ops.EPI_BIAS_BF16, out0=self.dh_small)
            if i > 0:
                self._inject_dmap(i - 1)
            if fuse and i > 0:
                pb, bb = f"blocks.{i - 1}.", br[2 * i - 1]
                self._before_overwrite("dY")
                ops.layernorm_bwd_branch(self.dh_small, xin, self.P(pre + "norm1.weight"), a["mean1"], a["rstd1"], dx,
                                         self.G(pre + "norm1.weight"), self.G(pre + "norm1.bias"), M, D, None,
                                         self.P(pb + "gamma_2") if (pb + "gamma_2") in self.segs else None, dY, None,
                                         self.G(pb + "mlp.fc2.bias"), rowmask=bb.rowmask, keep_prob=bb.keep_prob,
                                         rows_per_sample=T, in_map=ba.cmap, out_map=bb.cmap, dropout=self._drop(2 * i - 1))
            elif ba.n > 0:
                ops.layernorm_bwd(self.dh_small, xin, self.P(pre + "norm1.weight"), a["mean1"], a["rstd1"], dx,
                                  self.G(pre + "norm1.weight"), self.G(pre + "norm1.bias"), ba.rows, D, accumulate=True,
                                  row_idx=ba.ridx)
            self._bucket_ready(self.depth - i)
        self._backward_embed(c, B, M)

    def _backward_embed(self, c, B, M):
        D, T, L = self.D, self.T, self.L
        dx = self.dx
        dpos = self._drop(2 * self.depth)
        if dpos is not None:
            ops.dropout_rows(dpos, dx, M, D)
        if self.has_pos:
            if self.accumulate_grads:
                self.G("pos_embed").view(T, D).add_(dx[:M].view(B, T, D).sum(0))
            else:
                self.G("pos_embed").view(T, D).copy_(dx[:M].view(B, T, D).sum(0))
        ops.embed_bwd(dx, c["mask"], B, L, D, self.dYpe, self.G("cls_token"),
                      self.G("mask_token") if "mask_token" in self.segs else self.zero_vec)
        self._on_side(lambda: self._wgrad(self.dYpe, self.patches, B * L, D, self.Kpe, "patch_embed.proj.weight",
                                          bias_grads=((self.G("patch_embed.proj.bias"), 0, D),)))
        self._side_join()
        if self.grad_hook:
            self.grad_hook(self.depth + 1)

    def grad_norm(self, end=None):
        n = self.nflat if end is None else end
        ops.grad_norm(self.flat_g[:n], n, self.gnorm, self.gn_ws)
        return self.gnorm

    def weights_updated(self, end=None):
        if end is None or end >= self.nflat:
            self.weights_dirty = True
        elif not self.weights_dirty:
            assert end <= self.head_end, "partial weight update: the head bucket only (no transposed copies to refresh)"
            ops.cast_f32_bf16(self.flat_p[:end], self.flat_w16[:end], end)
            self.w16_version += 1

    def adamw_step(self, m, v, lr, wd, step, betas=(0.9, 0.95), eps=1e-8, max_norm=0.0):
        if not (self.overlap_optimizer and self.head_kind == "mlm" and not self.fwd_two_streams):
            self.wait_optimizer()
            ops.adamw(self.flat_p, self.flat_g, m, v, self.nflat, self.wd_flags, lr, betas[0], betas[1], eps, wd, step,
                      gnorm=self.gnorm, max_norm=max_norm or 0.0)
            self.weights_dirty = True
            return
        self.wait_optimizer()
        if self._tdesc is None:
            self._build_transpose_descs()
        if self._opt_stream is None:
            self._opt_stream = torch.cuda.Stream(device=self.dev)
            self._opt_events = {b[0]: torch.cuda.Event() for b in self.buckets}
            self._opt_events["__done__"] = torch.cuda.Event()
            self._opt_start = torch.cuda.Event()
        main, st = torch.cuda.current_stream(), self._opt_stream
        self._opt_start.record(main)
        with torch.cuda.stream(st):
            st.wait_event(self._opt_start)
            for name, b0, b1 in reversed(self.buckets):
                if b1 == b0:
                    self._opt_events[name].record(st)
                    continue
                ops.adamw(self.flat_p[b0:b1], self.flat_g[b0:b1], m[b0:b1], v[b0:b1], b1 - b0,
                          self.wd_flags[b0 // ALIGN: b1 // ALIGN], lr, betas[0], betas[1], eps, wd, step,
                          gnorm=self.gnorm, max_norm=max_norm or 0.0)
                ops.cast_f32_bf16(self.flat_p[b0:b1], self.flat_w16[b0:b1], b1 - b0)
                self._opt_events[name].record(st)
            for name, (k0, n, p0, tiles) in self._tbucket.items():
                ops.transpose_cast_batched(self._tdesc[k0:k0 + n], self._tprefix_loc[p0:p0 + n + 1], n, tiles)
            self._opt_events["__done__"].record(st)
        self._opt_ev = self._opt_events
        self._opt_done = self._opt_events["__done__"]
        self.weights_dirty = False
        self.w16_version += 1

    def _wait_params(self, bucket):
        if self._opt_ev is not None:
            torch.cuda.current_stream().wait_event(self._opt_ev[bucket])

    def wait_optimizer(self):
        if self._opt_done is not None:
            torch.cuda.current_stream().wait_event(self._opt_done)
            self._opt_ev = None
            self._opt_done = None
```

Before: 7788 samples/sec.

## Merge per-block bias folds, gemv and layerscale grads into one side-stream kernel

Adds a block_vectors kernel that in one launch folds the fc1 bias colsum copies, runs the proj gemv into v_bias with its proj-bias accumulate, and computes the layerscale gamma gradient. It moves these small launches off the critical stream onto the side stream. Per-block scratch (bias_scr, cs_ws) becomes one depth-sized buffer that is cleared together with the small gradients, so the per-step zero and the ping-pong zeroing go away. The fc2 dgrad GEMM now skips padded rows in its colsum via colsum_rows instead of zeroing the dY padding first. The cost is more scratch memory, and correctness now relies on side-stream ordering and the new zero-plan range.

```diff
diff --git a/include/memhip.h b/include/memhip.h
--- a/include/memhip.h
+++ b/include/memhip.h
@@ -173,7 +173,7 @@
   float* colsum;
   const int32_t* sample_map;
   int32_t colsum_copies;
-  int32_t reserved0;
+  int32_t colsum_rows;
   const memhip_dropout_t* dropout;
 } memhip_gemm_args_t;
 int memhip_gemm_bf16_nt(const memhip_gemm_args_t* args, memhip_stream_t stream);
@@ -252,6 +252,25 @@
 int memhip_layerscale_grad(const void* W_bf16, int64_t ldw, const float* dW, int64_t lddw, const float* bias,
                            const float* dbias, const float* gamma, int N, int K, float* dgamma,
                            memhip_stream_t stream);
+
+struct memhip_block_vectors_args {
+  const void* gemv_W; int64_t gemv_ldw;
+  const float* x;
+  float* y;
+  float* x_acc;
+  int32_t gemv_n, gemv_k;
+  const float* fold_ws;
+  float* fold_out;
+  int32_t fold_copies, fold_n;
+  const void* W; int64_t ldw;
+  const float* dW; int64_t lddw;
+  const float* bias; const float* dbias;
+  const float* gamma;
+  float* dgamma;
+  int32_t N, K;
+};
+typedef struct memhip_block_vectors_args memhip_block_vectors_args_t;
+int memhip_block_vectors(const memhip_block_vectors_args_t* args, memhip_stream_t stream);
 
 typedef struct memhip_branch {
   const void* y; int64_t ldy;
diff --git a/mem_amd/csrc/block_vectors.hip b/mem_amd/csrc/block_vectors.hip
--- /dev/null
+++ b/mem_amd/csrc/block_vectors.hip
@@ -0,0 +1,108 @@
+#include "common.h"
+
+namespace {
+
+using namespace memhip;
+
+typedef __attribute__((ext_vector_type(4))) __bf16 bf16x4;
+typedef __attribute__((ext_vector_type(8))) __bf16 bf16x8;
+typedef memhip_block_vectors_args_t Args;
+
+__device__ __forceinline__ float wsum(float v) {
+  for (int o = 32; o > 0; o >>= 1) v += __shfl_xor(v, o);
+  return v;
+}
+
+__global__ __launch_bounds__(256) void block_vectors_kernel(Args a, int nmain) {
+  __shared__ float red[4][4];
+  const int lane = threadIdx.x & 63, wave = threadIdx.x >> 6;
+  if ((int)blockIdx.x >= nmain) {
+    const int n = ((int)blockIdx.x - nmain) * 256 + threadIdx.x;
+    if (n >= a.fold_n) return;
+    float s = 0.f;
+    for (int k = 0; k < a.fold_copies; ++k) s += a.fold_ws[(long long)k * a.fold_n + n];
+    a.fold_out[n] += s;
+    return;
+  }
+  const int n0 = blockIdx.x * 4;
+  if (a.gemv_W) {
+    const __bf16* W = (const __bf16*)a.gemv_W;
+    const float* x = a.x;
+    const int n = n0 + wave, K = a.gemv_k;
+    if (n < a.gemv_n) {
+      float s = 0.f;
+      for (int k = lane * 8; k < K; k += 512) {
+        const bf16x8 w = *reinterpret_cast<const bf16x8*>(W + (long long)n * a.gemv_ldw + k);
+        const float4 p = *reinterpret_cast<const float4*>(x + k), q = *reinterpret_cast<const float4*>(x + k + 4);
+        s += (float)w[0] * p.x + (float)w[1] * p.y + (float)w[2] * p.z + (float)w[3] * p.w + (float)w[4] * q.x +
+             (float)w[5] * q.y + (float)w[6] * q.z + (float)w[7] * q.w;
+      }
+      for (int o = 32; o > 0; o >>= 1) s += __shfl_xor(s, o);
+      if (lane == 0) a.y[n] += s;
+    }
+    if (a.x_acc && threadIdx.x < 4 && n0 + (int)threadIdx.x < K) a.x_acc[n0 + threadIdx.x] += x[n0 + threadIdx.x];
+  }
+  if (!a.gamma || n0 >= a.N) return;
+  const __bf16* W = (const __bf16*)a.W;
+  const int N = a.N, K = a.K;
+  float s[4] = {0.f, 0.f, 0.f, 0.f};
+  for (int k0 = 0; k0 < K; k0 += 4096) {
+#pragma unroll
+    for (int c = 0; c < 4; ++c) {
+      const int n = n0 + c < N ? n0 + c : N - 1;
+      const __bf16* wr = W + (long long)n * a.ldw;
+      const float* gr = a.dW + (long long)n * a.lddw;
+#pragma unroll
+      for (int u = 0; u < 4; ++u) {
+        const int k = k0 + u * 1024 + (int)threadIdx.x * 4;
+        if (k < K) {
+          const bf16x4 w = *reinterpret_cast<const bf16x4*>(wr + k);
+          const float4 g = *reinterpret_cast<const float4*>(gr + k);
+          s[c] += (float)w[0] * g.x + (float)w[1] * g.y + (float)w[2] * g.z + (float)w[3] * g.w;
+        }
+      }
+    }
+  }
+#pragma unroll
+  for (int c = 0; c < 4; ++c) {
+    const float t = wsum(s[c]);
+    if (lane == 0) red[wave][c] = t;
+  }
+  __syncthreads();
+  if (threadIdx.x < 4 && n0 + (int)threadIdx.x < N) {
+    const int n = n0 + threadIdx.x;
+    float t = (red[0][threadIdx.x] + red[1][threadIdx.x]) + (red[2][threadIdx.x] + red[3][threadIdx.x]);
+    if (a.bias && a.dbias) t += a.bias[n] * a.dbias[n];
+    const float g = a.gamma[n];
+    a.dgamma[n] = g != 0.f ? t / g : 0.f;
+  }
+}
+
+}
+
+extern "C" int memhip_block_vectors(const memhip_block_vectors_args_t* args, memhip_stream_t stream) {
+  MEMHIP_REQUIRE(args, "block_vectors: null args");
+  const Args& a = *args;
+  int nmain = 0, nfold = 0;
+  if (a.gemv_W) {
+    MEMHIP_REQUIRE(a.gemv_n >= 0 && a.gemv_k >= 0 && a.gemv_k % 8 == 0 && a.gemv_ldw % 8 == 0,
+                   "block_vectors: gemv_k and gemv_ldw must be multiples of 8");
+    MEMHIP_REQUIRE(a.x && a.y, "block_vectors: null pointer (gemv)");
+    if (a.gemv_n > 0 && a.gemv_k > 0) nmain = cdiv(a.gemv_n > a.gemv_k ? a.gemv_n : a.gemv_k, 4);
+  }
+  if (a.fold_ws) {
+    MEMHIP_REQUIRE(a.fold_copies >= 1 && a.fold_n > 0, "block_vectors: bad fold shape");
+    MEMHIP_REQUIRE(a.fold_out, "block_vectors: null pointer (fold)");
+    nfold = cdiv(a.fold_n, 256);
+  }
+  if (a.gamma) {
+    MEMHIP_REQUIRE(a.N >= 0 && a.K > 0 && a.K % 4 == 0 && a.ldw % 4 == 0 && a.lddw % 4 == 0, "block_vectors: bad scale shape");
+    MEMHIP_REQUIRE(a.W && a.dW && a.dgamma && (!a.bias == !a.dbias), "block_vectors: null pointer (scale)");
+    MEMHIP_REQUIRE(!(a.gemv_W && a.x_acc && a.x_acc == a.dbias) || a.gemv_k == a.N,
+                   "block_vectors: x_acc is dbias, so gemv_k=%d must equal N=%d", a.gemv_k, a.N);
+    if (cdiv(a.N, 4) > nmain) nmain = cdiv(a.N, 4);
+  }
+  if (nmain + nfold == 0) return MEMHIP_OK;
+  hipLaunchKernelGGL(block_vectors_kernel, dim3(nmain + nfold), dim3(256), 0, as_stream(stream), a, nmain);
+  return check_launch("block_vectors");
+}
diff --git a/mem_amd/csrc/fp32_path.hip b/mem_amd/csrc/fp32_path.hip
--- a/mem_amd/csrc/fp32_path.hip
+++ b/mem_amd/csrc/fp32_path.hip
@@ -423,6 +423,7 @@
   __builtin_memset(&p, 0, sizeof(p));
   __builtin_memcpy(&p, a, offsetof(memhip_gemm_args_t, dropout));
   if (a->dropout) return fail(MEMHIP_EUNSUPPORTED, "gemm_f32: dropout is not part of the fp32 parity path");
+  if (p.colsum_rows != 0) return fail(MEMHIP_EUNSUPPORTED, "gemm_f32: colsum_rows is not part of the fp32 parity path");
   MEMHIP_REQUIRE(p.M >= 0 && p.N > 0 && p.K > 0, "gemm_f32: bad shape M=%d N=%d K=%d", p.M, p.N, p.K);
   if (p.M == 0) return MEMHIP_OK;
   MEMHIP_REQUIRE(p.A && p.B && p.K % 4 == 0 && p.lda % 4 == 0 && p.ldb % 4 == 0 && ((uintptr_t)p.A & 15) == 0 &&
diff --git a/mem_amd/csrc/gemm.hip b/mem_amd/csrc/gemm.hip
--- a/mem_amd/csrc/gemm.hip
+++ b/mem_amd/csrc/gemm.hip
@@ -1,3 +1,4 @@
+#include <climits>
 #include <cstddef>
 #include "common.h"
 #include "gemm_epilogue.hpp"
@@ -169,6 +170,8 @@
   __builtin_memset(&p, 0, sizeof(p));
   __builtin_memcpy(&p, a, offsetof(memhip_gemm_args_t, dropout));
   MEMHIP_REQUIRE(p.M >= 0 && p.N > 0 && p.K > 0, "gemm: bad shape M=%d N=%d K=%d", p.M, p.N, p.K);
+  MEMHIP_REQUIRE(p.colsum_rows >= 0, "gemm: colsum_rows=%d must not be negative", p.colsum_rows);
+  if (p.colsum_rows == 0) p.colsum_rows = INT_MAX;
   if (p.M == 0) return MEMHIP_OK;
   MEMHIP_REQUIRE(p.K % BK == 0, "gemm: K=%d must be a multiple of %d", p.K, BK);
   MEMHIP_REQUIRE(p.A && p.B, "gemm: null operand");
@@ -217,6 +220,7 @@
     p.aux = (const char*)p.aux + r * p.ldaux * (epi_resid(p.epilogue) ? 4 : 2);
   p.M = rows;
   p.m_base = row0;
+  p.colsum_rows -= row0;
   return p;
 }
 
diff --git a/mem_amd/csrc/gemm_epilogue.hpp b/mem_amd/csrc/gemm_epilogue.hpp
--- a/mem_amd/csrc/gemm_epilogue.hpp
+++ b/mem_amd/csrc/gemm_epilogue.hpp
@@ -71,7 +71,7 @@
     __bf16 y = (__bf16)v;
     if (n < p.colscale_n) y = (__bf16)((float)y * p.colscale);
     reinterpret_cast<__bf16*>(p.out0)[(long long)m * p.ldo0 + n] = y;
-    if (p.colsum) atomicAdd(colsum_base(p) + n, (float)y);
+    if (p.colsum && m < p.colsum_rows) atomicAdd(colsum_base(p) + n, (float)y);
   } else if constexpr (EPI == MEMHIP_EPI_BIAS_GELU) {
     const __bf16 h = (__bf16)(acc + bias_n);
     reinterpret_cast<__bf16*>(p.out0)[(long long)m * p.ldo0 + n] = h;
@@ -85,7 +85,7 @@
     const float g = (float)reinterpret_cast<const _Float16*>(p.aux)[(long long)m * p.ldaux + n];
     const __bf16 o = (__bf16)(da * g);
     reinterpret_cast<__bf16*>(p.out0)[(long long)m * p.ldo0 + n] = o;
-    if (p.colsum) atomicAdd(colsum_base(p) + n, (float)o);
+    if (p.colsum && m < p.colsum_rows) atomicAdd(colsum_base(p) + n, (float)o);
   } else if constexpr (EPI == MEMHIP_EPI_RESIDUAL) {
     const __bf16 y = (__bf16)(acc + bias_n);
     if (p.out0) reinterpret_cast<__bf16*>(p.out0)[(long long)m * p.ldo0 + n] = y;
@@ -118,7 +118,7 @@
     const float h = (float)reinterpret_cast<const __bf16*>(p.aux)[(long long)m * p.ldaux + n];
     const __bf16 o = (__bf16)(da * gelu_grad_f(h));
     reinterpret_cast<__bf16*>(p.out0)[(long long)m * p.ldo0 + n] = o;
-    if (p.colsum) atomicAdd(colsum_base(p) + n, (float)o);
+    if (p.colsum && m < p.colsum_rows) atomicAdd(colsum_base(p) + n, (float)o);
   } else if constexpr (EPI == MEMHIP_EPI_F32) {
     float* o = reinterpret_cast<float*>(p.out0) + (long long)m * p.ldo0 + n;
     *o = p.accumulate ? (*o + acc) : acc;
@@ -304,11 +304,12 @@
       for (int k = 0; k < 4; ++k) y[k] = pack_bf16x2(unpack_bf16x2(y[k]) * splat2(p.colscale));
     }
     if (p.colsum) {
+      const bool summed = m < p.colsum_rows;
 #pragma unroll
       for (int k = 0; k < 4; ++k) {
         const ef32x2 f = unpack_bf16x2(y[k]);
-        cs[2 * k] += f.x;
-        cs[2 * k + 1] += f.y;
+        cs[2 * k] += summed ? f.x : 0.f;
+        cs[2 * k + 1] += summed ? f.y : 0.f;
       }
     }
 #pragma unroll
@@ -332,11 +333,12 @@
 #pragma unroll
     for (int k = 0; k < 4; ++k) out[k] = pack_bf16x2(unpack_bf16x2(pack_bf16x2(t[k])) * unpack_f16x2(h[k]));
     if (p.colsum) {
+      const bool summed = m < p.colsum_rows;
 #pragma unroll
       for (int k = 0; k < 4; ++k) {
         const ef32x2 f = unpack_bf16x2(out[k]);
-        cs[2 * k] += f.x;
-        cs[2 * k + 1] += f.y;
+        cs[2 * k] += summed ? f.x : 0.f;
+        cs[2 * k + 1] += summed ? f.y : 0.f;
       }
     }
   } else if constexpr (epi_resid(EPI)) {
@@ -384,11 +386,12 @@
       out[k] = pack_bf16x2(da * gelu_grad2(unpack_bf16x2(h[k])));
     }
     if (p.colsum) {
+      const bool summed = m < p.colsum_rows;
 #pragma unroll
       for (int k = 0; k < 4; ++k) {
         const ef32x2 f = unpack_bf16x2(out[k]);
-        cs[2 * k] += f.x;
-        cs[2 * k + 1] += f.y;
+        cs[2 * k] += summed ? f.x : 0.f;
+        cs[2 * k + 1] += summed ? f.y : 0.f;
       }
     }
   } else if constexpr (EPI == MEMHIP_EPI_F32) {
diff --git a/mem_amd/csrc/gemm_nt_plan.hpp b/mem_amd/csrc/gemm_nt_plan.hpp
--- a/mem_amd/csrc/gemm_nt_plan.hpp
+++ b/mem_amd/csrc/gemm_nt_plan.hpp
@@ -21,7 +21,7 @@
   float* colsum;
   const int* sample_map;
   int colsum_copies;
-  int reserved0;
+  int colsum_rows;
   int m_base;
 };
 
diff --git a/mem_amd/ops.py b/mem_amd/ops.py
--- a/mem_amd/ops.py
+++ b/mem_amd/ops.py
@@ -30,7 +30,7 @@
                 ("bias", vp), ("vec1", vp), ("resid", vp), ("ldr", i64),
                 ("aux", vp), ("ldaux", i64), ("rowmask", vp), ("keep_prob", f32),
                 ("colscale", f32), ("colscale_n", i32), ("rows_per_sample", i32), ("accumulate", i32),
-                ("colsum", vp), ("sample_map", vp), ("colsum_copies", i32), ("reserved0", i32),
+                ("colsum", vp), ("sample_map", vp), ("colsum_copies", i32), ("colsum_rows", i32),
                 ("dropout", vp)]
 
 
@@ -95,7 +95,8 @@
 
 def gemm_args(A, B, M, N, K, epi, out0=None, out1=None, bias=None, vec1=None, resid=None, aux=None,
               rowmask=None, keep_prob=1.0, colscale=1.0, colscale_n=0, rows_per_sample=1, accumulate=False, colsum=None,
-              lda=None, ldb=None, ldo0=None, ldo1=None, ldr=None, ldaux=None, sample_map=None, colsum_copies=0, dropout=None):
+              lda=None, ldb=None, ldo0=None, ldo1=None, ldr=None, ldaux=None, sample_map=None, colsum_copies=0, dropout=None,
+              colsum_rows=0):
     a = GemmArgs()
     a.A, a.B = _p(A), _p(B)
     a.lda = A.stride(0) if lda is None else lda
@@ -115,6 +116,7 @@
     a.colsum = _p(colsum)
     a.sample_map = _p(sample_map)
     a.colsum_copies = colsum_copies
+    a.colsum_rows = colsum_rows
     a.dropout = None if dropout is None else C.addressof(dropout)
     return a
 
@@ -221,6 +223,31 @@
           "gemv_bf16_acc")
 
 
+class BlockVectorsArgs(C.Structure):
+    _fields_ = [("gemv_W", vp), ("gemv_ldw", i64), ("x", vp), ("y", vp), ("x_acc", vp), ("gemv_n", i32), ("gemv_k", i32),
+                ("fold_ws", vp), ("fold_out", vp), ("fold_copies", i32), ("fold_n", i32),
+                ("W", vp), ("ldw", i64), ("dW", vp), ("lddw", i64), ("bias", vp), ("dbias", vp), ("gamma", vp), ("dgamma", vp),
+                ("N", i32), ("K", i32)]
+
+
+declare({"memhip_block_vectors": (i32, [C.POINTER(BlockVectorsArgs), vp])})
+
+
+def block_vectors(gemv=None, fold=None, scale=None):
+    a = BlockVectorsArgs()
+    if gemv is not None:
+        W, N, K, x, y, x_acc = gemv
+        a.gemv_W, a.gemv_ldw, a.x, a.y, a.x_acc, a.gemv_n, a.gemv_k = _p(W), W.stride(0), _p(x), _p(y), _p(x_acc), N, K
+    if fold is not None:
+        ws, copies, N, out = fold
+        a.fold_ws, a.fold_out, a.fold_copies, a.fold_n = _p(ws), _p(out), copies, N
+    if scale is not None:
+        W16, dW, bias, dbias, gamma, N, K, dgamma = scale
+        a.W, a.ldw, a.dW, a.lddw = _p(W16), W16.stride(0), _p(dW), dW.stride(0)
+        a.bias, a.dbias, a.gamma, a.dgamma, a.N, a.K = _p(bias), _p(dbias), _p(gamma), _p(dgamma), N, K
+    check(lib.memhip_block_vectors(C.byref(a), stream_ptr()), "block_vectors")
+
+
 CONV_MODES = ("bf16", "fp32", "fp16x2")
 _CONV_MODE = {torch.bfloat16: 0, torch.float32: 1, torch.float16: 2}
 _F16X2 = 2
diff --git a/mem_amd/vit_engine.py b/mem_amd/vit_engine.py
--- a/mem_amd/vit_engine.py
+++ b/mem_amd/vit_engine.py
@@ -130,6 +130,7 @@
         self._zero_plans = {}
         self.grad_hook = None
         self.hook_on_side = True
+        self.block_vector_launches = "merged"
         self.accumulate_grads = False
         self.overlap_optimizer = False
         self._opt_stream = None
@@ -199,8 +200,10 @@
         return names
 
     def _zero_small_grads(self, start=0):
-        key = ("zr", start)
+        scr = getattr(self, "vec_scr", None)
+        key = ("zr", start, None if scr is None else scr.data_ptr())
         if key not in self._zero_plans:
+            self._zero_plans = {k: v for k, v in self._zero_plans.items() if k[:2] != ("zr", start)}
             import numpy as np
             mats = sorted(self.segs[n] for n in self._matrix_grad_names())
             ranges, pos = [], start
@@ -213,6 +216,9 @@
                 pos = max(pos, end)
             if pos < self.nflat:
                 ranges.append((pos * 4, (self.nflat - pos) * 4))
+            if scr is not None:
+                assert (scr.data_ptr() - self.flat_g.data_ptr()) % 16 == 0 and scr.numel() % 4 == 0
+                ranges.append((scr.data_ptr() - self.flat_g.data_ptr(), scr.numel() * 4))
             arr = np.asarray(ranges, dtype=np.int64).reshape(-1, 2)
             self._zero_plans[key] = (torch.from_numpy(arr).to(self.dev), len(ranges), int(arr[:, 1].sum()) if len(ranges) else 0)
         dev, n, total = self._zero_plans[key]
@@ -266,7 +272,7 @@
         self.act = [self._act_set(B)]
         if self.head_kind != "mlm":
             self.zero_mask = torch.zeros(B * self.L, dtype=torch.uint8, device=dev)
-        for name in ("dx", "dY", "dh_small", "dY2", "dbig", "dqkv", "dao", "delta_ws", "_tn_ws", "bias_scr", "cs_ws", "dYpe"):
+        for name in ("dx", "dY", "dh_small", "dY2", "dbig", "dqkv", "dao", "delta_ws", "_tn_ws", "vec_scr", "bias_scr", "cs_ws", "dYpe"):
             if hasattr(self, name):
                 delattr(self, name)
         self._maps = []
@@ -295,8 +301,9 @@
         self.dao = z(Ma, D)
         self.delta_ws = e(2 * M + 4, self.heads, dt=f32)
         self._tn_ws = torch.empty(0, dtype=torch.uint8, device=dev)
-        self.bias_scr = torch.zeros(2, D, dtype=f32, device=dev)
-        self.cs_ws = torch.zeros(self.CS_COPIES, self.hidden, dtype=f32, device=dev)
+        self.vec_scr = torch.zeros(self.depth * (D + self.CS_COPIES * self.hidden), dtype=f32, device=dev)
+        self.bias_scr = self.vec_scr[: self.depth * D].view(self.depth, D)
+        self.cs_ws = self.vec_scr[self.depth * D:].view(self.depth, self.CS_COPIES, self.hidden)
         self.dYpe = e(B * self.L, D)
         self.B_stash = B
 
@@ -621,7 +628,33 @@
         for gv, c0, c1 in bias_grads:
             ops.colsum_bf16(dY[:, c0:c1], R, c1 - c0, gv)
 
-    def _wg_mlp(self, pre, a, has_g, R, dY):
+    def _merged_vectors(self):
+        if self.block_vector_launches not in ("merged", "separate"):
+            raise ValueError(f"block_vector_launches = {self.block_vector_launches!r}: 'merged' or 'separate'")
+        return self.block_vector_launches == "merged"
+
+    def _mlp_vectors(self, i, pre, has_g):
+        D, Hd = self.D, self.hidden
+        scale = (self.W16(pre + "mlp.fc2.weight", D, Hd), self.G(pre + "mlp.fc2.weight").view(D, Hd),
+                 self.P(pre + "mlp.fc2.bias"), self.G(pre + "mlp.fc2.bias"), self.P(pre + "gamma_2"), D, Hd,
+                 self.G(pre + "gamma_2")) if has_g else None
+        if self._merged_vectors():
+            ops.block_vectors(fold=(self.cs_ws[i], self.CS_COPIES, Hd, self.G(pre + "mlp.fc1.bias")), scale=scale)
+        elif has_g:
+            ops.layerscale_grad(*scale)
+
+    def _attn_vectors(self, i, pre, scale):
+        D = self.D
+        scale = (self.W16(pre + "attn.proj.weight", D, D), self.G(pre + "attn.proj.weight").view(D, D),
+                 self.P(pre + "attn.proj.bias"), self.G(pre + "attn.proj.bias"), self.P(pre + "gamma_1"), D, D,
+                 self.G(pre + "gamma_1")) if scale else None
+        if self._merged_vectors():
+            ops.block_vectors(gemv=(self.wT[i]["proj"], D, D, self.bias_scr[i], self.G(pre + "attn.v_bias"),
+                                    self.G(pre + "attn.proj.bias")), scale=scale)
+        elif scale:
+            ops.layerscale_grad(*scale)
+
+    def _wg_mlp(self, i, pre, a, has_g, R, dY):
         D, Hd = self.D, self.hidden
         both = int(self.wgrad_group) >= 2
         if both:
@@ -629,10 +662,7 @@
         else:
             self._wgrad(dY, a["a"], R, D, Hd, pre + "mlp.fc2.weight")
         self._side_read_done("dY")
-        if has_g:
-            ops.layerscale_grad(self.W16(pre + "mlp.fc2.weight", D, Hd), self.G(pre + "mlp.fc2.weight").view(D, Hd),
-                                self.P(pre + "mlp.fc2.bias"), self.G(pre + "mlp.fc2.bias"),
-                                self.P(pre + "gamma_2"), D, Hd, self.G(pre + "gamma_2"))
+        self._mlp_vectors(i, pre, has_g)
         if not both:
             self._wgrad(self.dbig, a["h2"], R, Hd, D, pre + "mlp.fc1.weight")
         self._side_read_done("dbig")
@@ -785,6 +815,16 @@
                        self.cur["M"], self.D, rowmask=ba.rowmask, keep_prob=ba.keep_prob, rows_per_sample=self.T,
                        out_map=ba.cmap, dropout=self._drop(2 * i))
 
+    def _fc2_dgrad(self, i, pre, a, rows, gemm_rows):
+        D, Hd = self.D, self.hidden
+        merged = self._merged_vectors()
+        if not merged and gemm_rows > rows:
+            ops.zero_(self.dY[rows:gemm_rows])
+        ops.gemm_nt(self.dY, self.wT[i]["fc2"], gemm_rows, Hd, D, self.epi_dgelu, out0=self.dbig, aux=a["hpre"],
+                    colsum=self.cs_ws[i], colsum_copies=self.CS_COPIES, colsum_rows=rows)
+        if not merged:
+            ops.colsum_fold(self.cs_ws[i], self.CS_COPIES, Hd, self.G(pre + "mlp.fc1.bias"))
+
     def _mlp_bwd_tail(self, i, a, pre, has_g, keep, tail, scr):
         D, Hd = self.D, self.hidden
         rows, Mm, rk = tail["rows"], tail["Mm"], tail["rowkeep"]
@@ -794,13 +834,9 @@
         self._before_overwrite("dY")
         ops.branch_bwd(self.dxc, None, self.P(pre + "gamma_2") if has_g else None, dY, None, self.G(pre + "mlp.fc2.bias"),
                        Mm, D, rowmask=rk, keep_prob=keep, rows_per_sample=1)
-        if Mp > Mm:
-            ops.zero_(dY[Mm:Mp])
         self._before_overwrite("dbig")
-        ops.gemm_nt(dY, self.wT[i]["fc2"], Mp, Hd, D, self.epi_dgelu, out0=self.dbig, aux=a["hpre"],
-                    colsum=self.cs_ws, colsum_copies=self.CS_COPIES)
-        ops.colsum_fold(self.cs_ws, self.CS_COPIES, Hd, self.G(pre + "mlp.fc1.bias"))
-        self._on_side(lambda: self._wg_mlp(pre, a, has_g, Mm, dY))
+        self._fc2_dgrad(i, pre, a, Mm, Mp)
+        self._on_side(lambda: self._wg_mlp(i, pre, a, has_g, Mm, dY))
         ops.gemm_nt(self.dbig, self.wT[i]["fc1"], Mp, D, Hd, ops.EPI_BIAS_BF16, out0=self.dh_small)
         ops.layernorm_bwd(self.dh_small, self.x[2 * i + 1], self.P(pre + "norm2.weight"), a["mean2"], a["rstd2"], dx,
                           self.G(pre + "norm2.weight"), self.G(pre + "norm2.bias"), Mm, D, accumulate=True, row_idx=rows)
@@ -812,7 +848,8 @@
         D, Hd, T = self.D, self.hidden, self.T
         dx, dY, dY2 = self.dx, self.dY, self.dY2
         self._bucket_ready(0)
-        ops.zero_(self.bias_scr)
+        if self.accumulate_grads:
+            ops.zero_(self.vec_scr)
         fuse = D <= 1024 and self.fuse_ln_branch
         self._inject_dmap(self.depth - 1)
         for i in reversed(range(self.depth)):
@@ -822,7 +859,7 @@
             xin, xmid = self.x[2 * i], self.x[2 * i + 1]
             has_g = (pre + "gamma_1") in self.segs
             table, dtable = self.table(i), self.dtable(i)
-            scr = self.bias_scr[i & 1]
+            scr = self.bias_scr[i]
             tail = c["tail"] if i == self.depth - 1 else None
             if tail is not None:
                 self._mlp_bwd_tail(i, a, pre, has_g, bm.keep_prob, tail, scr)
@@ -837,12 +874,8 @@
                     self._zero_grad_of(pre + "mlp.fc2.weight")
                 if bm.n > 0:
                     self._before_overwrite("dbig")
-                    if bm.gemm_rows > bm.rows:
-                        ops.zero_(dY[bm.rows:bm.gemm_rows])
-                    ops.gemm_nt(dY, self.wT[i]["fc2"], bm.gemm_rows, Hd, D, self.epi_dgelu, out0=self.dbig, aux=a["hpre"],
-                                colsum=self.cs_ws, colsum_copies=self.CS_COPIES)
-                    ops.colsum_fold(self.cs_ws, self.CS_COPIES, Hd, self.G(pre + "mlp.fc1.bias"))
-                    self._on_side(lambda: self._wg_mlp(pre, a, has_g, bm.rows, dY))
+                    self._fc2_dgrad(i, pre, a, bm.rows, bm.gemm_rows)
+                    self._on_side(lambda: self._wg_mlp(i, pre, a, has_g, bm.rows, dY))
                     ops.gemm_nt(self.dbig, self.wT[i]["fc1"], bm.gemm_rows, D, Hd, ops.EPI_BIAS_BF16, out0=self.dh_small)
                 if fuse:
                     self._before_overwrite("dY2")
@@ -862,17 +895,16 @@
                 self._zero_grad_of(pre + "attn.qkv.weight")
             if ba.n > 0:
                 ops.gemm_nt(dY2, self.wT[i]["proj"], ba.gemm_rows, D, D, ops.EPI_BIAS_BF16, out0=self.dao)
-            ops.gemv_acc(self.wT[i]["proj"], D, D, scr, self.G(pre + "attn.v_bias"),
-                         x_acc=self.G(pre + "attn.proj.bias"), zero=self.bias_scr[(i & 1) ^ 1])
+            if not self._merged_vectors():
+                ops.gemv_acc(self.wT[i]["proj"], D, D, scr, self.G(pre + "attn.v_bias"), x_acc=self.G(pre + "attn.proj.bias"))
+            elif ba.n == 0:
+                self._on_side(lambda: self._attn_vectors(i, pre, False))
             if ba.n > 0:
                 def wg_proj(grouped=False):
                     if not grouped:
                         self._wgrad(dY2, a["ao"], ba.rows, D, D, pre + "attn.proj.weight")
                     self._side_read_done("dY2")
-                    if has_g:
-                        ops.layerscale_grad(self.W16(pre + "attn.proj.weight", D, D), self.G(pre + "attn.proj.weight").view(D, D),
-                                            self.P(pre + "attn.proj.bias"), self.G(pre + "attn.proj.bias"),
-                                            self.P(pre + "gamma_1"), D, D, self.G(pre + "gamma_1"))
+                    self._attn_vectors(i, pre, has_g)
                 if not self.wgrad_group:
                     self._on_side(wg_proj)
                 self._before_overwrite("dqkv")
```

Result: no change. 7811 samples/sec (median of 6 runs) (+0.3%).
